# lmdu/pyfastx

Hardware: NVIDIA H100
Metric: index_build_GBps (higher is better)
Workload: dtype u8

## Files before the change

include/fxg.h:

```cpp
#ifndef FXG_H
#define FXG_H
#include <stdint.h>
#ifdef __cplusplus
extern "C" {
#endif

#define FXG_ABI_VERSION 2

enum {
    FXG_OK       = 0,
    FXG_ENODEV   = -1,
    FXG_ECUDA    = -2,
    FXG_EINVAL   = -3,
    FXG_ENOMEM   = -4,
    FXG_ECAP     = -5,
    FXG_EIO      = -6,
    FXG_EFORMAT  = -7
};


typedef struct fxg_fasta_row {
    int64_t boff;
    int64_t blen;
    int64_t slen;
    int64_t llen;
    int32_t dlen;
    int32_t nlen;
    uint8_t elen;
    uint8_t norm;
    uint8_t pad[6];
} fxg_fasta_row;

typedef struct fxg_fastq_row {
    int64_t soff;
    int64_t qoff;
    int64_t rlen;
    int32_t dlen;
    int32_t nlen;
} fxg_fastq_row;

typedef struct fxg_scan_stats {
    int64_t n_rows;
    int64_t n_lines;
    int64_t total_len;
    int64_t end_position;
    int64_t lead_lines;
    int64_t lead_bytes;
    int64_t lead_llen;
    int64_t reserved;
} fxg_scan_stats;

typedef struct fxg_shard_info {
    int64_t n_rows;
    int64_t n_lines;
    int64_t bytes;
    int64_t base_offset;
    int64_t end_position;
    int64_t edge_n;
    int64_t edge_off[3];
    int64_t edge_len[3];
    int64_t reserved[4];
} fxg_shard_info;

enum {
    FXG_SCAN_FULL_NAME = 1
};

enum {
    FXG_X_UPPER      = 1,
    FXG_X_REVERSE    = 2,
    FXG_X_COMPLEMENT = 4,
    FXG_X_RAW        = 8,
    FXG_X_WHOLE      = 16
};

typedef struct fxg_ctx  fxg_ctx;
typedef struct fxg_file fxg_file;
typedef struct fxg_comm fxg_comm;

int         fxg_abi_version(void);
const char *fxg_last_error(void);
int         fxg_device_count(void);
int         fxg_ctx_create(int device, fxg_ctx **out);
void        fxg_ctx_destroy(fxg_ctx *ctx);
int         fxg_ctx_set_stream(fxg_ctx *ctx, void *cuda_stream);
int         fxg_ctx_sync(fxg_ctx *ctx);
int         fxg_ctx_sm_count(fxg_ctx *ctx);

enum { FXG_PROF_SCAN = 0, FXG_PROF_FINALIZE = 1, FXG_PROF_GATHER = 2, FXG_PROF_PLAN = 3, FXG_PROF_PREFIX = 4,
       FXG_PROF_LINES = 5, FXG_PROF_SLOTS = 6 };
int         fxg_profile_enable(fxg_ctx *ctx, int on);
int         fxg_profile_last_ms(fxg_ctx *ctx, int slot, float *ms);
int64_t     fxg_ctx_launch_count(fxg_ctx *ctx);

int         fxg_host_alloc(int64_t nbytes, void **out);
void        fxg_host_free(void *p);

int      fxg_file_alloc(fxg_ctx *ctx, int64_t nbytes, fxg_file **out);
int      fxg_file_upload(fxg_ctx *ctx, fxg_file *f, int64_t dst_off, const void *host, int64_t nbytes);
int      fxg_file_from_host(fxg_ctx *ctx, const void *host, int64_t nbytes, fxg_file **out);
int      fxg_file_from_path(fxg_ctx *ctx, const char *path, fxg_file **out);
int      fxg_file_wrap(fxg_ctx *ctx, void *dev_ptr, int64_t nbytes, int64_t capacity, fxg_file **out);
int      fxg_file_download(fxg_ctx *ctx, const fxg_file *f, int64_t src_off, void *host, int64_t nbytes);
void    *fxg_file_devptr(const fxg_file *f);
int64_t  fxg_file_size(const fxg_file *f);
void     fxg_file_free(fxg_file *f);
void     fxg_pool_trim(void);

int fxg_fasta_scan(fxg_ctx *ctx, const fxg_file *f, int64_t base_offset, int flags,
                   fxg_fasta_row **d_rows_out, fxg_scan_stats *stats);

int fxg_fastq_scan(fxg_ctx *ctx, const fxg_file *f, int64_t base_offset,
                   fxg_fastq_row **d_rows_out, fxg_scan_stats *stats);

int fxg_scan_begin(fxg_ctx *ctx, const fxg_file *f, int mode, int64_t base_offset, int flags,
                   fxg_shard_info *d_info_out );
int fxg_shard_exchange(fxg_ctx *ctx, fxg_comm *comm, const void *d_send, void *d_recv, int64_t bytes_per_rank);
int fxg_scan_finish(fxg_ctx *ctx, const fxg_shard_info *d_all , int nranks, int rank,
                    void **d_rows_out, fxg_scan_stats *stats, fxg_shard_info *all_host);
int fxg_scan_sharded(fxg_ctx *ctx, fxg_comm *comm, const fxg_file *f, int mode, int64_t base_offset, int flags,
                     void **d_rows_out, fxg_scan_stats *stats, fxg_shard_info *all_host);

#define FXG_COMM_ID_BYTES 128
int  fxg_comm_unique_id(void *id_out);
int  fxg_comm_create(fxg_ctx *ctx, const void *id, int nranks, int rank, fxg_comm **out);
int  fxg_comm_nranks(const fxg_comm *comm);
int  fxg_comm_rank(const fxg_comm *comm);
int  fxg_comm_uses_p2p(const fxg_comm *comm);
int  fxg_comm_check(fxg_comm *comm);
void fxg_comm_destroy(fxg_comm *comm);

int fxg_split_point_dev(fxg_ctx *ctx, const fxg_file *f, int64_t from, int want_header, int64_t *pos);
int fxg_split_point_path(const char *path, int64_t from, int want_header, int64_t *pos, int64_t *file_size);
int fxg_file_from_path_range(fxg_ctx *ctx, const char *path, int64_t begin, int64_t end, fxg_file **out);
int fxg_file_slice(fxg_ctx *ctx, const fxg_file *src, int64_t begin, int64_t end, fxg_file **out);

int fxg_rows_download(fxg_ctx *ctx, const void *d_rows, int64_t n_rows, int row_bytes, void *host_rows);
int fxg_rows_upload(fxg_ctx *ctx, const void *host_rows, int64_t n_rows, int row_bytes, void **d_rows_out);
void fxg_dev_free(void *d_ptr);

int fxg_fasta_build_index_host(fxg_ctx *ctx, const void *host_buf, int64_t nbytes, int flags,
                               fxg_fasta_row *rows, int64_t rows_cap, fxg_scan_stats *stats);
int fxg_fastq_build_index_host(fxg_ctx *ctx, const void *host_buf, int64_t nbytes,
                               fxg_fastq_row *rows, int64_t rows_cap, fxg_scan_stats *stats);

int fxg_extract_plan_dev(fxg_ctx *ctx, const int64_t *d_s, const int64_t *d_e, int64_t nq,
                         int64_t *d_out_off, int64_t *total_bytes );
int fxg_extract_dev(fxg_ctx *ctx, const fxg_file *f, const fxg_fasta_row *d_rows, int64_t n_rows,
                    const int64_t *d_row_id, const int64_t *d_s, const int64_t *d_e,
                    const int32_t *d_flags, int64_t nq,
                    const int64_t *d_out_off, uint8_t *d_out, int64_t *d_acgt );
int fxg_extract_host(fxg_ctx *ctx, const fxg_file *f, const fxg_fasta_row *d_rows, int64_t n_rows,
                     const int64_t *row_id, const int64_t *s, const int64_t *e, const int32_t *flags,
                     int64_t nq, int64_t *out_off_host, uint8_t *out_host, int64_t out_cap,
                     int64_t *acgt_host );

int fxg_extract_one_host(fxg_ctx *ctx, const fxg_file *f, const fxg_fasta_row *d_rows, int64_t n_rows,
                         int64_t row_id, int64_t s, int64_t e, int32_t flags, uint8_t *out_host, int64_t out_cap);

int fxg_composition_host(fxg_ctx *ctx, const fxg_file *f, const fxg_fasta_row *d_rows, int64_t n_rows,
                         const int64_t *row_id, const int64_t *s, const int64_t *e, const int32_t *flags,
                         int64_t nq, int64_t *hist_host);

int fxg_reads_dev(fxg_ctx *ctx, const fxg_file *f, const fxg_fastq_row *d_rows, int64_t n_rows,
                  const int64_t *d_ids, int64_t nq, int32_t flags,
                  int64_t *d_out_off, uint8_t *d_seq_out, uint8_t *d_qual_out, int64_t out_cap,
                  int64_t *total_bytes);
int fxg_reads_host(fxg_ctx *ctx, const fxg_file *f, const fxg_fastq_row *d_rows, int64_t n_rows,
                   const int64_t *ids, int64_t nq, int32_t flags,
                   int64_t *out_off_host, uint8_t *seq_host, uint8_t *qual_host, int64_t out_cap);

int fxg_read_one_host(fxg_ctx *ctx, const fxg_file *f, const fxg_fastq_row *d_rows, int64_t n_rows, int64_t read_id,
                      int which, int32_t flags, int64_t rlen, uint8_t *out_host, int64_t out_cap);

int fxg_bgzf_members_host(const void *host_buf, int64_t nbytes, int64_t *cmp_off, int64_t *ucmp_off,
                          int64_t cap, int64_t *n_members, int64_t *total_uncompressed);
int fxg_inflate_members_dev(fxg_ctx *ctx, const fxg_file *compressed, const int64_t *d_cmp_off,
                            const int64_t *d_ucmp_off, int64_t n_members, uint8_t *d_out, int64_t out_cap,
                            int32_t *d_status);
int fxg_file_from_bgzf_host(fxg_ctx *ctx, const void *host_buf, int64_t nbytes, fxg_file **out,
                            int64_t *n_members_out);

typedef struct fxg_gzindex {
    int64_t  compressed_size, uncompressed_size;
    uint32_t spacing, window_size;
    int64_t  npoints;
    const int64_t *cmp_offset;
    const int64_t *uncmp_offset;
    const uint8_t *bits;
    const uint8_t *has_data;
    const uint8_t *windows;
} fxg_gzindex;
typedef struct fxg_comp_row { int64_t seqid, abc, num; } fxg_comp_row;
typedef struct fxg_fastq_meta { int64_t a, c, g, t, n, maxlen, minlen, minqs, maxqs, phred; } fxg_fastq_meta;
int fxg_fxi_write_fasta(const char *path, const fxg_fasta_row *rows, int64_t n_rows, const uint8_t *names,
                        const int64_t *name_off, int64_t total_slen, const fxg_gzindex *gz,
                        const fxg_comp_row *comp, int64_t n_comp);
int fxg_fxi_write_fastq(const char *path, const fxg_fastq_row *rows, int64_t n_rows, const uint8_t *names,
                        const int64_t *name_off, int64_t n_lines, int64_t total_size, const fxg_gzindex *gz,
                        const fxg_fastq_meta *meta);

typedef struct fxg_gzip_result fxg_gzip_result;
int            fxg_gzip_inflate_host(const void *comp, int64_t nbytes, uint32_t spacing , fxg_gzip_result **out);
const uint8_t *fxg_gzip_data(const fxg_gzip_result *r, int64_t *size);
int            fxg_gzip_index(const fxg_gzip_result *r, fxg_gzindex *gz);
void           fxg_gzip_free(fxg_gzip_result *r);
int            fxg_file_from_gzip_points_host(fxg_ctx *ctx, const void *host_buf, int64_t nbytes, const fxg_gzindex *gz,
                                              fxg_file **out);

int  fxg_fasta_composition(fxg_ctx *ctx, const fxg_file *f, const fxg_fasta_row *d_rows, int64_t n_rows,
                           int64_t base_offset, fxg_comp_row **out, int64_t *n_out, int64_t *total );
int  fxg_fastq_stats(fxg_ctx *ctx, const fxg_file *f, const fxg_fastq_row *d_rows, int64_t n_rows,
                     int64_t base_offset, int trailing_seq, fxg_fastq_meta *out);
void fxg_free_host(void *p);

typedef struct fxg_nametab fxg_nametab;
int     fxg_nametab_build(const uint8_t *names, const int64_t *name_off, int64_t n, fxg_nametab **out);
int64_t fxg_nametab_find(const fxg_nametab *t, const uint8_t *name, int64_t len);
int     fxg_nametab_lookup(const fxg_nametab *t, const uint8_t *q, const int64_t *q_off, int64_t nq, int64_t *ids_out);
void    fxg_nametab_free(fxg_nametab *t);

int fxg_bgzf_compress_host(const void *data, int64_t nbytes, int level, uint8_t **out, int64_t *out_len);

int fxg_synth_fasta_dev(fxg_ctx *ctx, uint64_t seed, const int64_t *d_lengths, const int64_t *d_rec_off,
                        int64_t n_records, int64_t first_record, int width, uint8_t *d_out);
int fxg_synth_fastq_dev(fxg_ctx *ctx, uint64_t seed, int64_t n_reads, int64_t first_read, int read_len,
                        const int64_t *d_rec_off, uint8_t *d_out);

#ifdef __cplusplus
}
#endif
#endif
```

pyfastx_b200/_cabi.py:

```python
import ctypes as C
import os
import re

import numpy as np

_HERE = os.path.dirname(os.path.abspath(__file__))
LIB_PATH = os.environ.get("FXG_LIB_PATH") or os.path.join(_HERE, "libfxg.so")
HEADER_PATH = os.path.join(os.path.dirname(_HERE), "include", "fxg.h")

FASTA_ROW = np.dtype([("boff", "<i8"), ("blen", "<i8"), ("slen", "<i8"), ("llen", "<i8"),
                      ("dlen", "<i4"), ("nlen", "<i4"), ("elen", "u1"), ("norm", "u1"),
                      ("pad", "u1", (6,))])
FASTQ_ROW = np.dtype([("soff", "<i8"), ("qoff", "<i8"), ("rlen", "<i8"),
                      ("dlen", "<i4"), ("nlen", "<i4")])

FXG_OK, FXG_ENODEV, FXG_ECUDA, FXG_EINVAL, FXG_ENOMEM, FXG_ECAP, FXG_EIO, FXG_EFORMAT = 0, -1, -2, -3, -4, -5, -6, -7
SCAN_FULL_NAME = 1
X_UPPER, X_REVERSE, X_COMPLEMENT, X_RAW, X_WHOLE = 1, 2, 4, 8, 16


class ScanStats(C.Structure):
    _fields_ = [("n_rows", C.c_int64), ("n_lines", C.c_int64), ("total_len", C.c_int64),
                ("end_position", C.c_int64), ("lead_lines", C.c_int64), ("lead_bytes", C.c_int64),
                ("lead_llen", C.c_int64), ("reserved", C.c_int64)]


class ShardInfo(C.Structure):
    _fields_ = [("n_rows", C.c_int64), ("n_lines", C.c_int64), ("bytes", C.c_int64), ("base_offset", C.c_int64),
                ("end_position", C.c_int64), ("edge_n", C.c_int64), ("edge_off", C.c_int64 * 3),
                ("edge_len", C.c_int64 * 3), ("reserved", C.c_int64 * 4)]


SHARD_INFO = np.dtype([("n_rows", "<i8"), ("n_lines", "<i8"), ("bytes", "<i8"), ("base_offset", "<i8"),
                       ("end_position", "<i8"), ("edge_n", "<i8"), ("edge_off", "<i8", (3,)), ("edge_len", "<i8", (3,)),
                       ("reserved", "<i8", (4,))])
COMM_ID_BYTES = 128


class GzIndex(C.Structure):
    _fields_ = [("compressed_size", C.c_int64), ("uncompressed_size", C.c_int64), ("spacing", C.c_uint32),
                ("window_size", C.c_uint32), ("npoints", C.c_int64), ("cmp_offset", C.c_void_p),
                ("uncmp_offset", C.c_void_p), ("bits", C.c_void_p), ("has_data", C.c_void_p), ("windows", C.c_void_p)]


class FastqMeta(C.Structure):
    _fields_ = [(k, C.c_int64) for k in ("a", "c", "g", "t", "n", "maxlen", "minlen", "minqs", "maxqs", "phred")]


COMP_ROW = np.dtype([("seqid", "<i8"), ("abc", "<i8"), ("num", "<i8")])


class FxgError(RuntimeError):
    def __init__(self, code, msg):
        super().__init__("libfxg error %d: %s" % (code, msg))
        self.code = code


class NoDeviceError(FxgError):
    pass


vp, i64, i32, u64 = C.c_void_p, C.c_int64, C.c_int, C.c_uint64
P = C.POINTER

SIGNATURES = {
    "fxg_abi_version": (i32, []),
    "fxg_last_error": (C.c_char_p, []),
    "fxg_device_count": (i32, []),
    "fxg_ctx_create": (i32, [i32, P(vp)]),
    "fxg_ctx_destroy": (None, [vp]),
    "fxg_ctx_set_stream": (i32, [vp, vp]),
    "fxg_ctx_sync": (i32, [vp]),
    "fxg_ctx_sm_count": (i32, [vp]),
    "fxg_profile_enable": (i32, [vp, i32]),
    "fxg_profile_last_ms": (i32, [vp, i32, P(C.c_float)]),
    "fxg_ctx_launch_count": (i64, [vp]),
    "fxg_host_alloc": (i32, [i64, P(vp)]),
    "fxg_host_free": (None, [vp]),
    "fxg_file_alloc": (i32, [vp, i64, P(vp)]),
    "fxg_file_upload": (i32, [vp, vp, i64, vp, i64]),
    "fxg_file_from_host": (i32, [vp, vp, i64, P(vp)]),
    "fxg_file_from_path": (i32, [vp, C.c_char_p, P(vp)]),
    "fxg_file_wrap": (i32, [vp, vp, i64, i64, P(vp)]),
    "fxg_file_download": (i32, [vp, vp, i64, vp, i64]),
    "fxg_file_devptr": (vp, [vp]),
    "fxg_file_size": (i64, [vp]),
    "fxg_file_free": (None, [vp]),
    "fxg_pool_trim": (None, []),
    "fxg_fasta_scan": (i32, [vp, vp, i64, i32, P(vp), P(ScanStats)]),
    "fxg_fastq_scan": (i32, [vp, vp, i64, P(vp), P(ScanStats)]),
    "fxg_scan_begin": (i32, [vp, vp, i32, i64, i32, vp]),
    "fxg_shard_exchange": (i32, [vp, vp, vp, vp, i64]),
    "fxg_scan_finish": (i32, [vp, vp, i32, i32, P(vp), P(ScanStats), vp]),
    "fxg_scan_sharded": (i32, [vp, vp, vp, i32, i64, i32, P(vp), P(ScanStats), vp]),
    "fxg_comm_unique_id": (i32, [vp]),
    "fxg_comm_create": (i32, [vp, vp, i32, i32, P(vp)]),
    "fxg_comm_nranks": (i32, [vp]),
    "fxg_comm_rank": (i32, [vp]),
    "fxg_comm_uses_p2p": (i32, [vp]),
    "fxg_comm_check": (i32, [vp]),
    "fxg_comm_destroy": (None, [vp]),
    "fxg_split_point_dev": (i32, [vp, vp, i64, i32, P(i64)]),
    "fxg_split_point_path": (i32, [C.c_char_p, i64, i32, P(i64), P(i64)]),
    "fxg_file_from_path_range": (i32, [vp, C.c_char_p, i64, i64, P(vp)]),
    "fxg_file_slice": (i32, [vp, vp, i64, i64, P(vp)]),
    "fxg_rows_download": (i32, [vp, vp, i64, i32, vp]),
    "fxg_rows_upload": (i32, [vp, vp, i64, i32, P(vp)]),
    "fxg_dev_free": (None, [vp]),
    "fxg_fasta_build_index_host": (i32, [vp, vp, i64, i32, vp, i64, P(ScanStats)]),
    "fxg_fastq_build_index_host": (i32, [vp, vp, i64, vp, i64, P(ScanStats)]),
    "fxg_extract_plan_dev": (i32, [vp, vp, vp, i64, vp, P(i64)]),
    "fxg_extract_dev": (i32, [vp, vp, vp, i64, vp, vp, vp, vp, i64, vp, vp, vp]),
    "fxg_extract_host": (i32, [vp, vp, vp, i64, vp, vp, vp, vp, i64, vp, vp, i64, vp]),
    "fxg_extract_one_host": (i32, [vp, vp, vp, i64, i64, i64, i64, i32, vp, i64]),
    "fxg_composition_host": (i32, [vp, vp, vp, i64, vp, vp, vp, vp, i64, vp]),
    "fxg_reads_dev": (i32, [vp, vp, vp, i64, vp, i64, i32, vp, vp, vp, i64, P(i64)]),
    "fxg_reads_host": (i32, [vp, vp, vp, i64, vp, i64, i32, vp, vp, vp, i64]),
    "fxg_read_one_host": (i32, [vp, vp, vp, i64, i64, i32, i32, i64, vp, i64]),
    "fxg_bgzf_members_host": (i32, [vp, i64, vp, vp, i64, P(i64), P(i64)]),
    "fxg_inflate_members_dev": (i32, [vp, vp, vp, vp, i64, vp, i64, vp]),
    "fxg_file_from_bgzf_host": (i32, [vp, vp, i64, P(vp), P(i64)]),
    "fxg_fxi_write_fasta": (i32, [C.c_char_p, vp, i64, vp, vp, i64, vp, vp, i64]),
    "fxg_fxi_write_fastq": (i32, [C.c_char_p, vp, i64, vp, vp, i64, i64, vp, vp]),
    "fxg_gzip_inflate_host": (i32, [vp, i64, C.c_uint32, P(vp)]),
    "fxg_gzip_data": (vp, [vp, P(i64)]),
    "fxg_gzip_index": (i32, [vp, P(GzIndex)]),
    "fxg_gzip_free": (None, [vp]),
    "fxg_file_from_gzip_points_host": (i32, [vp, vp, i64, P(GzIndex), P(vp)]),
    "fxg_fasta_composition": (i32, [vp, vp, vp, i64, i64, P(vp), P(i64), vp]),
    "fxg_fastq_stats": (i32, [vp, vp, vp, i64, i64, i32, P(FastqMeta)]),
    "fxg_free_host": (None, [vp]),
    "fxg_nametab_build": (i32, [vp, vp, i64, P(vp)]),
    "fxg_nametab_find": (i64, [vp, C.c_char_p, i64]),
    "fxg_nametab_lookup": (i32, [vp, vp, vp, i64, vp]),
    "fxg_nametab_free": (None, [vp]),
    "fxg_bgzf_compress_host": (i32, [vp, i64, i32, P(vp), P(i64)]),
    "fxg_synth_fasta_dev": (i32, [vp, u64, vp, vp, i64, i64, i32, vp]),
    "fxg_synth_fastq_dev": (i32, [vp, u64, i64, i64, i32, vp, vp]),
}

_lib = None


def declared_symbols():
    with open(HEADER_PATH) as f:
        text = re.sub(r"/\*.*?\*/", "", f.read(), flags=re.S)
    return sorted(set(re.findall(r"\b(fxg_[a-z0-9_]+)\s*\(", text)))


def lib():
    global _lib
    if _lib is None:
        if not os.path.exists(LIB_PATH):
            raise FxgError(FXG_ENODEV, "libfxg.so not built (run pyfastx_b200/csrc/build.sh or "
                                       "__graft_entry__.build()); there is no CPU fallback")
        L = C.CDLL(LIB_PATH)
        for name, (res, args) in SIGNATURES.items():
            fn = getattr(L, name)
            fn.restype = res
            fn.argtypes = args
        _lib = L
    return _lib


def check(rc):
    if rc != FXG_OK:
        msg = lib().fxg_last_error().decode("utf-8", "replace")
        raise (NoDeviceError if rc == FXG_ENODEV else FxgError)(rc, msg)
    return rc


def ptr(a):
    if a is None:
        return None
    if isinstance(a, int):
        return a
    if isinstance(a, np.ndarray):
        return a.ctypes.data
    if hasattr(a, "data_ptr"):
        return a.data_ptr()
    raise TypeError("cannot take a pointer of %r" % type(a))
```

pyfastx_b200/csrc/fxg_scan.cu:

```cuda
#include "fxg_common.cuh"
#include <stdlib.h>
#include <string.h>
#include <limits.h>

namespace fxg {

#ifndef FXG_MARK_MINB
#define FXG_MARK_MINB 6
#endif
constexpr int REGION   = 2048;
constexpr int SEGCAP   = 128;
constexpr int MARK_WARPS = 8;
constexpr int PS_THREADS = 256, PS_PER_THREAD = 16, PS_BLOCK = PS_THREADS * PS_PER_THREAD;
constexpr int64_t NOPOS = INT64_MIN / 4;
constexpr uint32_t E_POS = 0x07ffu, E_CR = 1u << 14, E_HDR = 1u << 15;

struct __align__(16) FastaTmp {
    int64_t  boff;
    int64_t  lineidx;
    int64_t  llen;
    uint64_t S;
    uint64_t evmax;
    uint64_t evminc;
    uint32_t D;
    int32_t  dlen;
    int32_t  nlen;
    uint32_t elen;
};
static_assert(sizeof(FastaTmp) == 64, "FastaTmp layout");

struct ScanTotals {
    uint64_t nl;
    uint64_t hdr;
    int64_t  n_eff;
    uint64_t sum_len;
    int64_t  lead_lines, lead_bytes, lead_llen;
    int64_t  first_line;
    int64_t  nrows;
    int64_t  row0;
    int64_t  n_owned;
    int64_t  total_lines;
    int64_t  pad[4];
};
static_assert(sizeof(ScanTotals) == 128, "ScanTotals layout");
static_assert(sizeof(fxg_shard_info) == 128, "fxg_shard_info layout");

struct ScanParams;
struct ScanParams {
    const uint8_t *file;
    int64_t   n;
    int64_t   capacity;
    int64_t   nreg;
    int64_t   base_offset;
    int64_t   first_line;
    int       flags;
    uint2    *rc;
    uint4    *rec2;
    uint16_t *seg;
    uint8_t  *cut;
    ulonglong2 *ex;
    ulonglong2 *bs;
    ScanTotals *totals;
    FastaTmp *tmp;
    int64_t   tmp_cap;
    fxg_fastq_row *qrows;
    int64_t   qrows_cap;
    const ScanParams *self;
};

__device__ __forceinline__ uint4 ld_stream16(const uint8_t *p) {
    uint4 v;
    asm volatile("ld.global.nc.L1::no_allocate.v4.u32 {%0, %1, %2, %3}, [%4];"
                 : "=r"(v.x), "=r"(v.y), "=r"(v.z), "=r"(v.w) : "l"(p));
    return v;
}

#ifndef FXG_MARK_CUT
#define FXG_MARK_CUT 0
#endif
#ifndef FXG_CUT_WORDS
#define FXG_CUT_WORDS 6
#endif
__device__ __forceinline__ uint32_t swz_unit(uint32_t u);
template <int V> __device__ __forceinline__ uint32_t region_byte(const uint8_t *sb, uint32_t p);
template <int V>
__device__ __forceinline__ uint32_t name_cut_smem(const uint8_t *sb, uint32_t a) {
    uint32_t M = 0;
#pragma unroll
    for (int k = 0; k < FXG_CUT_WORDS; ++k) {
        const uint32_t wq = min((a >> 2) + (uint32_t)k, (uint32_t)(REGION / 4 - 1));
        const uint32_t w = reinterpret_cast<const uint32_t *>(sb)[V == 2 ? ((swz_unit(wq >> 2) << 2) | (wq & 3u)) : wq];
        const uint32_t lt = ~((((w & 0x7f7f7f7fu) + 0x5f5f5f5fu) | w)) & 0x80808080u;
        M |= ((lt * 0x00204081u) >> 28) << (4 * k);
    }
    M &= 0xffffffffu << (a & 3u);
    if (!M) return 255u;
    const uint32_t p = (a & ~3u) + (uint32_t)(__ffs(M) - 1);
    if (p >= (uint32_t)REGION) return 255u;
    if (p >= ((a >> 2) + (uint32_t)FXG_CUT_WORDS) * 4u) return 255u;
    const uint32_t b = region_byte<V>(sb, p);
    if (b == ' ') return p - a;
    if (b == '\n' || b == 0u) return 254u;
    if (b == '\r' && p + 1u < (uint32_t)REGION && region_byte<V>(sb, p + 1u) == '\n') return 254u;
    return 255u;
}

#ifndef FXG_MARK_V_FASTA
#define FXG_MARK_V_FASTA 1
#endif
#ifndef FXG_MARK_V_FASTQ
#define FXG_MARK_V_FASTQ 2
#endif
#ifndef FXG_MARK_RPW
#define FXG_MARK_RPW 1
#endif
__device__ __forceinline__ uint32_t swz_unit(uint32_t u) { return u ^ ((u >> 3) & 7u); }
template <int V>
__device__ __forceinline__ uint32_t region_byte(const uint8_t *sb, uint32_t p) {
    return V == 2 ? sb[(swz_unit(p >> 4) << 4) | (p & 15u)] : sb[p];
}

template <int MODE, int V>
__global__ void __launch_bounds__(MARK_WARPS * 32, FXG_MARK_MINB) mark_kernel(const ScanParams P) {
    __shared__ uint4    s_data[MARK_WARPS * (REGION / 16) + (FXG_MARK_CUT ? 2 : 0)];
    __shared__ uint16_t s_ent[MARK_WARPS][SEGCAP];
    const int lane = threadIdx.x & 31, warp = threadIdx.x >> 5;
    const int64_t r0 = ((int64_t)blockIdx.x * MARK_WARPS + warp) * FXG_MARK_RPW;
    if (r0 >= P.nreg) return;
    const uint32_t lt_mask = (1u << lane) - 1u;
    const int64_t n = P.n;
    const uint8_t *file = P.file;
    const uint32_t k0a = reg_const(0x0a0a0a0au), k7f = reg_const(0x7f7f7f7fu), k80 = reg_const(0x80808080u);

    auto load_region = [&](int64_t rr, uint4 (&vv)[4]) {
        const int64_t base = rr * REGION;
        if (base + REGION <= n) {
            const uint8_t *src = file + base + lane * 16;
#pragma unroll
            for (int j = 0; j < 4; ++j) vv[j] = ld_stream16(src + j * 512);
        } else {
#pragma unroll
            for (int j = 0; j < 4; ++j) {
                const int64_t o = base + j * 512 + lane * 16;
                if (o + 16 <= n) { vv[j] = ld_stream16(file + o); continue; }
                const bool virt = n > 0 && file[n - 1] != '\n';
                uint32_t w[4] = {0, 0, 0, 0};
                for (int i = 0; i < 16; ++i) {
                    const int64_t x = o + i;
                    const uint32_t b = x < n ? file[x] : ((virt && x == n) ? 0x0au : 0u);
                    w[i >> 2] |= b << ((i & 3) * 8);
                }
                vv[j] = make_uint4(w[0], w[1], w[2], w[3]);
            }
        }
    };
    uint4 vn[4];
    load_region(r0, vn);
#pragma unroll 1
    for (int it = 0; it < FXG_MARK_RPW; ++it) {
    const int64_t r = r0 + it;
    if (r >= P.nreg) break;
    const int64_t base = r * REGION;
    uint4 v[4] = {vn[0], vn[1], vn[2], vn[3]};
    if (it + 1 < FXG_MARK_RPW && r + 1 < P.nreg) load_region(r + 1, vn);
    uint32_t nlc = 0;
    uint16_t *ent = s_ent[warp];

    if constexpr (V == 2) {
    uint4 *sd = s_data + warp * (REGION / 16);
#pragma unroll
    for (int j = 0; j < 4; ++j) sd[swz_unit((uint32_t)(j * 32 + lane))] = v[j];
    __syncwarp();
    uint32_t lo = 0, hi = 0;
#pragma unroll
    for (int i = 0; i < 4; ++i) {
        const uint4 x = sd[swz_unit((uint32_t)(4 * lane + i))];
        const uint32_t w4[4] = {x.x, x.y, x.z, x.w};
#pragma unroll
        for (int c = 0; c < 4; ++c) {
            const uint32_t f = byte_eq_mask_r(w4[c], k0a, k7f, k80);
            const uint32_t nib = (f * 0x00204081u) >> 28;
            const int k = 4 * i + c;
            if (k < 8) lo = nib * (1u << (4 * k)) + lo;
            else hi = nib * (1u << (4 * (k - 8))) + hi;
        }
    }
    {
        const uint32_t c = (uint32_t)(__popc(lo) + __popc(hi));
        const uint32_t b1 = __ballot_sync(0xffffffffu, c >= 1u), b2 = __ballot_sync(0xffffffffu, c >= 2u);
        const uint32_t b3 = __ballot_sync(0xffffffffu, c >= 3u);
        const uint32_t pbase = (uint32_t)lane * 64u;
        if (!b3) {
            const uint32_t idx = (uint32_t)(__popc(b1 & lt_mask) + __popc(b2 & lt_mask));
            nlc = (uint32_t)(__popc(b1) + __popc(b2));
            if (c) {
                const uint32_t p1 = lo ? (uint32_t)(__ffs(lo) - 1) : 32u + (uint32_t)(__ffs(hi) - 1);
                if (idx < (uint32_t)SEGCAP) ent[idx] = (uint16_t)(pbase + p1);
                if (c >= 2u) {
                    if (lo) lo &= lo - 1u; else hi &= hi - 1u;
                    const uint32_t p2 = lo ? (uint32_t)(__ffs(lo) - 1) : 32u + (uint32_t)(__ffs(hi) - 1);
                    if (idx + 1u < (uint32_t)SEGCAP) ent[idx + 1u] = (uint16_t)(pbase + p2);
                }
            }
        } else {
            uint32_t incl = c;
#pragma unroll
            for (int d = 1; d < 32; d <<= 1) {
                const uint32_t o2 = __shfl_up_sync(0xffffffffu, incl, d);
                if (lane >= d) incl += o2;
            }
            nlc = __shfl_sync(0xffffffffu, incl, 31);
            uint32_t idx = incl - c;
            while (lo) { if (idx < (uint32_t)SEGCAP) ent[idx] = (uint16_t)(pbase + (uint32_t)(__ffs(lo) - 1)); lo &= lo - 1u; ++idx; }
            while (hi) { if (idx < (uint32_t)SEGCAP) ent[idx] = (uint16_t)(pbase + 32u + (uint32_t)(__ffs(hi) - 1)); hi &= hi - 1u; ++idx; }
        }
    }
    __syncwarp();
    } else {
    uint32_t m[4];
    int cmax = 0;
#pragma unroll
    for (int j = 0; j < 4; ++j) {
        s_data[warp * (REGION / 16) + j * 32 + lane] = v[j];
        m[j] = chunk_eq_mask_r(v[j], k0a, k7f, k80);
        cmax = max(cmax, __popc(m[j]));
    }
    const bool any2 = __any_sync(0xffffffffu, cmax >= 2);
    const bool multi = any2 && __any_sync(0xffffffffu, cmax >= 3);
    if (!any2) {
#pragma unroll
        for (int j = 0; j < 4; ++j) {
            const uint32_t bn = __ballot_sync(0xffffffffu, m[j] != 0);
            if (m[j]) {
                const uint32_t idx = nlc + __popc(bn & lt_mask);
                if (idx < (uint32_t)SEGCAP) ent[idx] = (uint16_t)(j * 512 + lane * 16 + chunk_bit_to_off(__ffs(m[j]) - 1));
            }
            nlc += __popc(bn);
        }
    } else if (!multi) {
#pragma unroll
        for (int j = 0; j < 4; ++j) {
            const int c = __popc(m[j]);
            const uint32_t bn1 = __ballot_sync(0xffffffffu, c >= 1);
            const uint32_t bn2 = __ballot_sync(0xffffffffu, c >= 2);
            if (c) {
                const uint32_t idx = nlc + __popc(bn1 & lt_mask) + __popc(bn2 & lt_mask);
                const int xo = j * 512 + lane * 16;
                int oa = chunk_bit_to_off(__ffs(m[j]) - 1);
                if (c == 2) {
                    const uint32_t m2 = m[j] & (m[j] - 1);
                    const int ob = chunk_bit_to_off(__ffs(m2) - 1);
                    const int hi = max(oa, ob);
                    oa = min(oa, ob);
                    if (idx + 1 < (uint32_t)SEGCAP) ent[idx + 1] = (uint16_t)(xo + hi);
                }
                if (idx < (uint32_t)SEGCAP) ent[idx] = (uint16_t)(xo + oa);
            }
            nlc += __popc(bn1) + __popc(bn2);
        }
    }
    if (multi) {
        nlc = 0;
#pragma unroll 1
        for (int j = 0; j < 4; ++j) {
            uint32_t mj = 0;
#pragma unroll
            for (int jj = 0; jj < 4; ++jj) if (jj == j) mj = m[jj];
            const uint32_t c = (uint32_t)__popc(mj);
            uint32_t incl = c;
#pragma unroll
            for (int d = 1; d < 32; d <<= 1) {
                const uint32_t o2 = __shfl_up_sync(0xffffffffu, incl, d);
                if (lane >= d) incl += o2;
            }
            uint32_t idx = nlc + incl - c;
#pragma unroll 1
            for (int w = 0; w < 4; ++w) {
                uint32_t mw = mj & (0x80808080u >> w);
                while (mw) {
                    if (idx < (uint32_t)SEGCAP) ent[idx] = (uint16_t)(j * 512 + lane * 16 + chunk_bit_to_off(__ffs(mw) - 1));
                    mw &= mw - 1;
                    ++idx;
                }
            }
            nlc += __shfl_sync(0xffffffffu, incl, 31);
        }
    }
    __syncwarp();
    }

    const uint8_t *sb = reinterpret_cast<const uint8_t *>(s_data + warp * (REGION / 16));
    uint32_t hc = 0;
    if (nlc <= (uint32_t)SEGCAP) {
        uint16_t *dst = P.seg + r * SEGCAP;
        const uint32_t nround = (nlc + 15u) & ~15u;
        uint32_t imask = 0, hmask = 0;
        for (uint32_t k0 = 0; k0 < nround; k0 += 32) {
            const uint32_t k = k0 + lane;
            uint32_t e = 0, cutv = 255u;
            if (k < nlc) {
                const uint32_t pos = ent[k];
                e = pos;
                if (FXG_MARK_CUT && MODE == 1 && pos + 2u < (uint32_t)REGION && region_byte<V>(sb, pos + 1u) == '@') cutv = name_cut_smem<V>(sb, pos + 2u);
                if (MODE == 0) {
                    const uint32_t next = pos < (uint32_t)(REGION - 1) ? region_byte<V>(sb, pos + 1u)
                                                                      : (base + REGION < n ? (uint32_t)file[base + REGION] : 0u);
                    if (next == '>') e |= E_HDR;
                } else {
                    const uint32_t prev = pos > 0 ? region_byte<V>(sb, pos - 1u) : (base > 0 ? (uint32_t)file[base - 1] : 0u);
                    if (prev == '\r') e |= E_CR;
                }
            }
            if (MODE == 0) {
                const uint32_t hb = __ballot_sync(0xffffffffu, (e & E_HDR) != 0);
                hc += __popc(hb);
                if (k0 == 0) {
                    const uint32_t e1 = __shfl_up_sync(0xffffffffu, e, 1), e2 = __shfl_up_sync(0xffffffffu, e, 2);
                    const bool it = lane >= 2 && k < nlc &&
                                    (((e1 | e2) & E_HDR) != 0 || (e & E_POS) - (e1 & E_POS) != (e1 & E_POS) - (e2 & E_POS));
                    imask = __ballot_sync(0xffffffffu, it);
                    hmask = hb;
                }
            }
            if (k < nround) dst[k] = (uint16_t)e;
            if (FXG_MARK_CUT && MODE == 1) P.cut[r * SEGCAP + k] = (uint8_t)cutv;
            if (k < nlc) ent[k] = (uint16_t)e;
        }
        __syncwarp();
        if (lane == 0) {
            const uint32_t last = nlc >= 1 ? ent[nlc - 1] : 0u, prev = nlc >= 2 ? ent[nlc - 2] : 0u;
            P.rc[r] = make_uint2(nlc | (hc << 16), last | (prev << 16));
            if (MODE == 0) {
                const uint32_t f0 = nlc >= 1 ? ent[0] : 0u, f1 = nlc >= 2 ? ent[1] : 0u;
                P.rec2[r] = make_uint4(f0 | (f1 << 16), nlc > 32u ? 0xffffffffu : imask, hmask, 0u);
            }
        }
    } else {
        if (MODE == 0) {
            uint32_t myh = 0;
            for (int x = lane; x < REGION; x += 32)
                if (region_byte<V>(sb, (uint32_t)x) == '\n') {
                    const uint32_t next = x < REGION - 1 ? region_byte<V>(sb, (uint32_t)x + 1u) : (base + REGION < n ? (uint32_t)file[base + REGION] : 0u);
                    myh += next == '>';
                }
            hc = __reduce_add_sync(0xffffffffu, myh);
        }
        if (lane == 0) {
            P.rc[r] = make_uint2(nlc | (hc << 16), 0u);
            if (MODE == 0) P.rec2[r] = make_uint4(0u, 0xffffffffu, 0u, 0u);
        }
    }
    __syncwarp();
    }
}

__global__ void __launch_bounds__(PS_THREADS) prefix_reduce_kernel(const uint2 *rc, ulonglong2 *bs) {
    __shared__ uint32_t sm[16];
    const uint4 *p = reinterpret_cast<const uint4 *>(rc + (size_t)blockIdx.x * PS_BLOCK + (size_t)threadIdx.x * PS_PER_THREAD);
    uint32_t a = 0, b = 0;
#pragma unroll
    for (int i = 0; i < PS_PER_THREAD / 2; ++i) {
        const uint4 q = p[i];
        a += (q.x & 0xffffu) + (q.z & 0xffffu);
        b += (q.x >> 16) + (q.z >> 16);
    }
    a = __reduce_add_sync(0xffffffffu, a);
    b = __reduce_add_sync(0xffffffffu, b);
    const int lane = threadIdx.x & 31, warp = threadIdx.x >> 5;
    if (lane == 0) { sm[warp] = a; sm[8 + warp] = b; }
    __syncthreads();
    if (threadIdx.x == 0) {
        uint64_t ta = 0, tb = 0;
        for (int w = 0; w < PS_THREADS / 32; ++w) { ta += sm[w]; tb += sm[8 + w]; }
        bs[blockIdx.x] = make_ulonglong2(ta, tb);
    }
}

__global__ void __launch_bounds__(1024) prefix_blocks_kernel(ulonglong2 *bs, int64_t nb, const uint8_t *file, int64_t n,
                                                             int mode, ScanTotals *tot) {
    __shared__ uint64_t s_a[32], s_b[32];
    __shared__ uint64_t s_ca, s_cb;
    const int lane = threadIdx.x & 31, warp = threadIdx.x >> 5;
    if (threadIdx.x == 0) { s_ca = 0; s_cb = (mode == 0 && n > 0 && file[0] == '>') ? 1u : 0u; }
    __syncthreads();
    for (int64_t b0 = 0; b0 < nb; b0 += 1024) {
        const int64_t i = b0 + threadIdx.x;
        const ulonglong2 v = i < nb ? bs[i] : make_ulonglong2(0, 0);
        uint64_t a = v.x, b = v.y;
#pragma unroll
        for (int d = 1; d < 32; d <<= 1) {
            const uint64_t oa = (uint64_t)shfl_up_i64((int64_t)a, d), ob = (uint64_t)shfl_up_i64((int64_t)b, d);
            if (lane >= d) { a += oa; b += ob; }
        }
        if (lane == 31) { s_a[warp] = a; s_b[warp] = b; }
        __syncthreads();
        uint64_t wa = 0, wb = 0;
        for (int w = 0; w < warp; ++w) { wa += s_a[w]; wb += s_b[w]; }
        const uint64_t ca = s_ca, cb = s_cb;
        if (i < nb) bs[i] = make_ulonglong2(ca + wa + a - v.x, cb + wb + b - v.y);
        __syncthreads();
        if (threadIdx.x == 1023) { s_ca = ca + wa + a; s_cb = cb + wb + b; }
        __syncthreads();
    }
    if (threadIdx.x == 0) {
        const bool virt = n > 0 && file[n - 1] != '\n';
        tot->nl = s_ca; tot->hdr = s_cb; tot->n_eff = n + (virt ? 1 : 0);
    }
}

__global__ void __launch_bounds__(PS_THREADS) prefix_expand_kernel(const uint2 *rc, const ulonglong2 *bs, ulonglong2 *ex,
                                                                 int64_t nreg) {
    __shared__ uint32_t s_a[PS_THREADS / 32], s_b[PS_THREADS / 32];
    const int lane = threadIdx.x & 31, warp = threadIdx.x >> 5;
    const size_t r0 = (size_t)blockIdx.x * PS_BLOCK + (size_t)threadIdx.x * PS_PER_THREAD;
    const uint4 *p = reinterpret_cast<const uint4 *>(rc + r0);
    uint32_t c[PS_PER_THREAD];
    uint32_t a = 0, b = 0;
#pragma unroll
    for (int i = 0; i < PS_PER_THREAD / 2; ++i) {
        const uint4 q = p[i];
        c[2 * i] = q.x; c[2 * i + 1] = q.z;
        a += (q.x & 0xffffu) + (q.z & 0xffffu);
        b += (q.x >> 16) + (q.z >> 16);
    }
    uint32_t ia = a, ib = b;
#pragma unroll
    for (int d = 1; d < 32; d <<= 1) {
        const uint32_t oa = __shfl_up_sync(0xffffffffu, ia, d), ob = __shfl_up_sync(0xffffffffu, ib, d);
        if (lane >= d) { ia += oa; ib += ob; }
    }
    if (lane == 31) { s_a[warp] = ia; s_b[warp] = ib; }
    __syncthreads();
    uint32_t wa = 0, wb = 0;
    for (int w = 0; w < warp; ++w) { wa += s_a[w]; wb += s_b[w]; }
    const ulonglong2 bb = bs[blockIdx.x];
    uint64_t ea = bb.x + wa + ia - a, eb = bb.y + wb + ib - b;
#pragma unroll
    for (int i = 0; i < PS_PER_THREAD; ++i) {
        if ((int64_t)(r0 + i) < nreg) ex[r0 + i] = make_ulonglong2(ea, eb);
        ea += c[i] & 0xffffu; eb += c[i] >> 16;
    }
}

__device__ __forceinline__ int64_t find_first_of2(const uint8_t *h, int64_t limit, uint32_t a4, uint32_t b4, int *which) {
    const int mis = (int)((uintptr_t)h & 3);
    const uint32_t *wp = reinterpret_cast<const uint32_t *>(h - mis);
    *which = 0;
    for (int64_t k = -mis; k < limit; k += 16, wp += 4) {
        const uint32_t w0 = wp[0], w1 = wp[1], w2 = wp[2], w3 = wp[3];
        uint32_t ma[4] = {byte_eq_mask(w0, a4), byte_eq_mask(w1, a4), byte_eq_mask(w2, a4), byte_eq_mask(w3, a4)};
        uint32_t mb[4] = {byte_eq_mask(w0, b4), byte_eq_mask(w1, b4), byte_eq_mask(w2, b4), byte_eq_mask(w3, b4)};
#pragma unroll
        for (int i = 0; i < 4; ++i) {
            uint32_t m = ma[i] | mb[i];
            const int64_t kk = k + 4 * i;
            if (kk < 0) m &= 0xffffffffu << (8 * (int)(-kk));
            if (m) {
                const int byte = (__ffs(m) - 1) >> 3;
                const int64_t pos = kk + byte;
                if (pos >= limit) return limit;
                *which = ((mb[i] >> (8 * byte)) & 0x80u) ? 2 : 1;
                return pos;
            }
        }
    }
    return limit;
}

struct Prev2 {
    int64_t  pos1, pos0;
    uint32_t h1, h0;
};

template <int MODE>
__device__ __forceinline__ uint32_t is_hdr_at(const ScanParams &P, int64_t x) {
    return (MODE == 0 && x < P.n && P.file[x] == '>') ? 1u : 0u;
}
__device__ __forceinline__ bool nl_at(const ScanParams &P, int64_t x) {
    return x < P.n ? P.file[x] == '\n' : (x == P.n && P.n > 0 && P.file[P.n - 1] != '\n');
}

template <int MODE>
__device__ __forceinline__ void do_line(const ScanParams &P, int64_t first_line, int64_t p, int64_t pm1, int64_t pm2, bool h1, bool h2,
                                        int64_t hcount, int64_t lineidx, bool cr, unsigned long long &my_size) {
    const uint8_t *file = P.file;
    const int64_t s = pm1 + 1;
    const int64_t L = p - pm1;
    if (MODE == 0) {
        const int64_t slot = hcount;
        if (h1) {
            const int elen = (p >= 1 && (p - 1 < P.n ? file[p - 1] : 0) == '\r') ? 2 : 1;
            const int64_t dlen = L - 1 - elen;
            int64_t nlen = dlen;
            if (!(P.flags & FXG_SCAN_FULL_NAME)) {
                nlen = 0;
                if (s + 1 + dlen + 20 <= P.capacity) {
                    int which;
                    nlen = find_first_of2(file + s + 1, dlen, 0x20202020u, 0x09090909u, &which);
                } else {
                    while (nlen < dlen) {
                        const uint8_t ch = file[s + 1 + nlen];
                        if (ch == ' ' || ch == '\t') break;
                        ++nlen;
                    }
                }
            }
            if (slot < P.tmp_cap) {
                FastaTmp *t = &P.tmp[slot];
                t->boff = P.base_offset + p + 1;
                t->lineidx = lineidx;
                t->dlen = (int32_t)dlen;
                t->nlen = (int32_t)nlen;
                t->elen = (uint32_t)elen;
            }
        } else if (slot < P.tmp_cap) {
            const bool prev_exists = pm1 >= 0;
            if (!prev_exists || h2) {
                P.tmp[slot].llen = L;
            } else {
                const int64_t prevL = pm1 - pm2;
                if (L != prevL) {
                    FastaTmp *t = &P.tmp[slot];
                    atomicAdd(&t->D, 1u);
                    atomicMax((unsigned long long *)&t->evmax, (unsigned long long)lineidx);
                    atomicMax((unsigned long long *)&t->evminc, ~(unsigned long long)lineidx);
                    atomicAdd((unsigned long long *)&t->S, (unsigned long long)(L - prevL));
                }
            }
        }
    } else {
        const int64_t gline = first_line + lineidx;
        const int ph = (int)(gline & 3);
        const int64_t row = (gline >> 2) - (first_line >> 2);
        const int64_t len = L - 1;
        if (ph == 1) {
            const int64_t rlen = (len > 0 && cr) ? len - 1 : len;
            my_size += (unsigned long long)rlen;
            if (row < P.qrows_cap) { P.qrows[row].soff = P.base_offset + s; P.qrows[row].rlen = rlen; }
        } else if (row < P.qrows_cap) {
            if (ph == 0) {
                int64_t l = len - 1;
                if (l > 0 && cr) --l;
                if (l < 0) l = 0;
                int64_t k = 0;
                if (s + 1 + l + 20 <= P.capacity) {
                    int which;
                    k = find_first_of2(file + s + 1, l, 0x20202020u, 0x00000000u, &which);
                    if (which == 2) k = l;
                } else {
                    for (; k < l; ++k) {
                        const uint8_t ch = file[s + 1 + k];
                        if (ch == 0) { k = l; break; }
                        if (ch == ' ') break;
                    }
                }
                *reinterpret_cast<int2 *>(&P.qrows[row].dlen) = make_int2((int)len, (int)k);
            } else if (ph == 3) {
                P.qrows[row].qoff = P.base_offset + s;
            }
        }
    }
}

template <int MODE>
__device__ __noinline__ Prev2 carry_walk(const ScanParams *Pg, int64_t r) {
    const ScanParams &P = *Pg;
    Prev2 cy;
    const int lane = threadIdx.x & 31;
    cy.pos1 = cy.pos0 = NOPOS; cy.h1 = cy.h0 = 0;
    int need = 2;
    auto push = [&](int64_t pos, uint32_t h) {
        if (need == 2) { cy.pos1 = pos; cy.h1 = h; } else { cy.pos0 = pos; cy.h0 = h; }
        --need;
    };
    int64_t q = r - 1;
    while (need > 0 && q >= 0) {
        const int64_t qq = q - lane;
        const uint32_t c = qq >= 0 ? (P.rc[qq].x & 0xffffu) : 0u;
        const uint32_t nz = __ballot_sync(0xffffffffu, c != 0);
        if (!nz) { q -= 32; continue; }
        const int f = __ffs(nz) - 1;
        q -= f;
        const int cq = (int)__shfl_sync(0xffffffffu, c, f);
        if (cq <= SEGCAP) {
            const uint16_t *sg = P.seg + q * SEGCAP;
            for (int i = cq - 1; i >= 0 && need > 0; --i) {
                const uint32_t e = sg[i];
                push(q * REGION + (int64_t)(e & E_POS), MODE == 0 ? (e >> 15) : 0u);
            }
        } else {
            for (int64_t x = q * REGION + REGION - 1; x >= q * REGION && need > 0; --x)
                if (nl_at(P, x)) push(x, is_hdr_at<MODE>(P, x + 1));
        }
        q -= 1;
    }
    if (need > 0) push(-1, is_hdr_at<MODE>(P, 0));
    return cy;
}

template <int MODE>
__device__ __noinline__ unsigned long long dense_region(const ScanParams *Pg, int64_t first_line, int64_t r, Prev2 cy,
                                                        ulonglong2 exv) {
    const ScanParams &P = *Pg;
    unsigned long long my_size = 0;
    const int lane = threadIdx.x & 31;
    const uint8_t *file = P.file;
    const int64_t b0 = r * REGION + lane * 64;
    uint32_t c = 0, h = 0;
    Prev2 inc; inc.pos1 = inc.pos0 = NOPOS; inc.h1 = inc.h0 = 0;
    for (int i = 0; i < 64; ++i) {
        const int64_t x = b0 + i;
        if (nl_at(P, x)) {
            const uint32_t hh = is_hdr_at<MODE>(P, x + 1);
            ++c; h += hh;
            inc.pos0 = inc.pos1; inc.h0 = inc.h1; inc.pos1 = x; inc.h1 = hh;
        }
    }
    uint32_t ic = c, ih = h;
    uint32_t icnt = c > 2 ? 2 : c;
#pragma unroll
    for (int d = 1; d < 32; d <<= 1) {
        const uint32_t oc = __shfl_up_sync(0xffffffffu, ic, d), oh = __shfl_up_sync(0xffffffffu, ih, d);
        const int64_t op1 = shfl_up_i64(inc.pos1, d), op0 = shfl_up_i64(inc.pos0, d);
        const uint32_t oh1 = __shfl_up_sync(0xffffffffu, inc.h1, d), oh0 = __shfl_up_sync(0xffffffffu, inc.h0, d);
        const uint32_t ocnt = __shfl_up_sync(0xffffffffu, icnt, d);
        if (lane >= d) {
            ic += oc; ih += oh;
            if (icnt == 0) { inc.pos1 = op1; inc.h1 = oh1; inc.pos0 = op0; inc.h0 = oh0; icnt = ocnt; }
            else if (icnt == 1 && ocnt >= 1) { inc.pos0 = op1; inc.h0 = oh1; icnt = 2; }
        }
    }
    Prev2 pv;
    pv.pos1 = shfl_up_i64(inc.pos1, 1); pv.pos0 = shfl_up_i64(inc.pos0, 1);
    pv.h1 = __shfl_up_sync(0xffffffffu, inc.h1, 1); pv.h0 = __shfl_up_sync(0xffffffffu, inc.h0, 1);
    uint32_t pcnt = __shfl_up_sync(0xffffffffu, icnt, 1);
    if (lane == 0) pcnt = 0;
    if (pcnt == 0) pv = cy;
    else if (pcnt == 1) { pv.pos0 = cy.pos1; pv.h0 = cy.h1; }
    int64_t idx = (int64_t)exv.x + (ic - c);
    int64_t hcount = (int64_t)exv.y + (ih - h);
    for (int i = 0; i < 64 && c; ++i) {
        const int64_t x = b0 + i;
        if (!nl_at(P, x)) continue;
        const bool cr = x > 0 && file[x - 1] == '\r';
        do_line<MODE>(P, first_line, x, pv.pos1, pv.pos0, pv.h1 != 0, pv.h0 != 0, hcount, idx, cr, my_size);
        const uint32_t hh = is_hdr_at<MODE>(P, x + 1);
        hcount += hh; ++idx;
        pv.pos0 = pv.pos1; pv.h0 = pv.h1; pv.pos1 = x; pv.h1 = hh;
    }
    return my_size;
}

template <int MODE>
__device__ __forceinline__ void region_batches(const ScanParams &P, int64_t first_line, int64_t r, int nl, Prev2 cy, ulonglong2 X,
                                               uint32_t E0, uint32_t E1, unsigned long long &my_size) {
    const int lane = threadIdx.x & 31;
    const uint32_t lt_mask = (1u << lane) - 1u;
    const int64_t base = r * REGION;
    const uint16_t *sg = P.seg + r * SEGCAP;
    int64_t hrun = (int64_t)X.y;
    for (int k0 = 0; k0 < nl; k0 += 32) {
        const int k = k0 + lane;
        const bool valid = k < nl;
        uint32_t e = k0 == 0 ? E0 : (k0 == 32 ? E1 : (valid ? (uint32_t)sg[k] : 0u));
        if (!valid) e = 0;
        const uint32_t hb = __ballot_sync(0xffffffffu, (e & E_HDR) != 0);
        const uint32_t e1 = __shfl_up_sync(0xffffffffu, e, 1), e2 = __shfl_up_sync(0xffffffffu, e, 2);
        if (valid) {
            int64_t pm1, pm2;
            bool h1, h2;
            if (lane >= 1) { pm1 = base + (e1 & E_POS); h1 = (e1 & E_HDR) != 0; } else { pm1 = cy.pos1; h1 = cy.h1 != 0; }
            if (lane >= 2) { pm2 = base + (e2 & E_POS); h2 = (e2 & E_HDR) != 0; }
            else if (lane == 1) { pm2 = cy.pos1; h2 = cy.h1 != 0; }
            else { pm2 = cy.pos0; h2 = cy.h0 != 0; }
            do_line<MODE>(P, first_line, base + (e & E_POS), pm1, pm2, h1, h2, hrun + __popc(hb & lt_mask), (int64_t)X.x + k,
                          (e & E_CR) != 0, my_size);
        }
        const uint32_t l31 = __shfl_sync(0xffffffffu, e, 31), l30 = __shfl_sync(0xffffffffu, e, 30);
        cy.pos1 = base + (l31 & E_POS); cy.h1 = (l31 >> 15) & 1u;
        cy.pos0 = base + (l30 & E_POS); cy.h0 = (l30 >> 15) & 1u;
        hrun += __popc(hb);
    }
}

template <int MODE>
__device__ __noinline__ unsigned long long full_region(const ScanParams *Pg, int64_t first_line, int64_t r) {
    const ScanParams &P = *Pg;
    unsigned long long my_size = 0;
    const int lane = threadIdx.x & 31;
    const int nl = (int)(P.rc[r].x & 0xffffu);
    if (nl == 0) return 0;
    const ulonglong2 X = P.ex[r];
    Prev2 cy = carry_walk<MODE>(Pg, r);
    if (MODE != 0) cy.h1 = cy.h0 = 0;
    if (nl <= SEGCAP) region_batches<MODE>(P, first_line, r, nl, cy, X, P.seg[r * SEGCAP + lane], P.seg[r * SEGCAP + 32 + lane], my_size);
    else my_size += dense_region<MODE>(Pg, first_line, r, cy, X);
    return my_size;
}

constexpr int LG = 4;

template <int MODE>
__global__ void __launch_bounds__(MARK_WARPS * 32) lines_kernel(const ScanParams P) {
    const int64_t first_line = MODE == 1 ? P.totals->first_line : 0;
    const int lane = threadIdx.x & 31;
    const int64_t r0 = ((int64_t)blockIdx.x * MARK_WARPS + (threadIdx.x >> 5)) * LG;
    if (r0 >= P.nreg) return;
    unsigned long long my_size = 0;

    const int64_t rq = r0 + (LG - 1) - lane;
    const uint2 A = rq >= 0 ? P.rc[rq] : make_uint2(0u, 0u);
    ulonglong2 X[LG];
    uint32_t E[LG][2];
#pragma unroll
    for (int i = 0; i < LG; ++i) {
        const int64_t r = r0 + i;
        X[i] = make_ulonglong2(0, 0); E[i][0] = E[i][1] = 0;
        if (r < P.nreg) {
            X[i] = P.ex[r];
            E[i][0] = P.seg[r * SEGCAP + lane];
            E[i][1] = P.seg[r * SEGCAP + 32 + lane];
        }
    }
    const uint32_t cntl = A.x & 0xffffu;
    const uint32_t nzall = __ballot_sync(0xffffffffu, cntl != 0);
    const bool window_hits_start = r0 + (LG - 1) - 31 <= 0;

#pragma unroll
    for (int i = 0; i < LG; ++i) {
        const int64_t r = r0 + i;
        const int me = LG - 1 - i;
        const int nl = (int)__shfl_sync(0xffffffffu, cntl, me);
        if (nl == 0) continue;

        Prev2 cy;
        cy.pos1 = cy.pos0 = NOPOS; cy.h1 = cy.h0 = 0;
        {
            bool slow = false;
            const uint32_t nz = nzall & ~((2u << me) - 1u);
            if (nz) {
                const int f1 = __ffs(nz) - 1;
                const uint32_t n1 = __shfl_sync(0xffffffffu, cntl, f1), y1 = __shfl_sync(0xffffffffu, A.y, f1);
                const int64_t b1 = (r0 + (LG - 1) - f1) * REGION;
                if (n1 > (uint32_t)SEGCAP) slow = true;
                else {
                    cy.pos1 = b1 + (y1 & E_POS); cy.h1 = (y1 >> 15) & 1u;
                    if (n1 >= 2) { cy.pos0 = b1 + ((y1 >> 16) & E_POS); cy.h0 = y1 >> 31; }
                    else {
                        const uint32_t nz2 = nz & ~(1u << f1);
                        if (nz2) {
                            const int f2 = __ffs(nz2) - 1;
                            const uint32_t n2 = __shfl_sync(0xffffffffu, cntl, f2), y2 = __shfl_sync(0xffffffffu, A.y, f2);
                            if (n2 > (uint32_t)SEGCAP) slow = true;
                            else { cy.pos0 = (r0 + (LG - 1) - f2) * REGION + (y2 & E_POS); cy.h0 = (y2 >> 15) & 1u; }
                        } else if (window_hits_start) { cy.pos0 = -1; cy.h0 = is_hdr_at<MODE>(P, 0); }
                        else slow = true;
                    }
                }
            } else if (window_hits_start) { cy.pos1 = -1; cy.h1 = is_hdr_at<MODE>(P, 0); }
            else slow = true;
            if (slow) cy = carry_walk<MODE>(P.self, r);
            if (MODE != 0) cy.h1 = cy.h0 = 0;
        }
        if (nl <= SEGCAP) region_batches<MODE>(P, first_line, r, nl, cy, X[i], E[i][0], E[i][1], my_size);
        else my_size += dense_region<MODE>(P.self, first_line, r, cy, X[i]);
    }

    if (MODE == 1) {
#pragma unroll
        for (int d = 16; d > 0; d >>= 1) my_size += (unsigned long long)shfl_down_i64((int64_t)my_size, d);
        if (lane == 0 && my_size) atomicAdd((unsigned long long *)&P.totals->sum_len, my_size);
    }
}

#ifndef FXG_FQ_PRELOAD
#define FXG_FQ_PRELOAD 0
#endif
#ifndef FXG_FQ_PAIRSTORE
#define FXG_FQ_PAIRSTORE 1
#endif
constexpr int RG = 8;
constexpr int RWIN = RG + 2;
static_assert(RWIN * REGION <= 32768, "window positions must fit 15 bits");

__global__ void __launch_bounds__(MARK_WARPS * 32) fastq_records_kernel(const ScanParams Pin) {
    __shared__ uint16_t s_flat[MARK_WARPS][RWIN * SEGCAP];
    __shared__ uint8_t  s_cut[MARK_WARPS][FXG_MARK_CUT ? RWIN * SEGCAP : 1];
    const ScanParams &P = Pin;
    const int64_t first_line = Pin.totals->first_line;
    const int lane = threadIdx.x & 31, warp = threadIdx.x >> 5;
    const int64_t r0 = ((int64_t)blockIdx.x * MARK_WARPS + warp) * RG;
    if (r0 >= P.nreg) return;
    unsigned long long my_size = 0;
    const uint8_t *file = P.file;

    const int64_t rl = r0 - 1 + lane;
    uint2 rec = make_uint2(0u, 0u);
    uint64_t exl = 0;
    if (lane <= RWIN && rl >= 0 && rl < P.nreg) { rec = P.rc[rl]; exl = P.ex[rl].x; }
    const uint32_t nll = rec.x & 0xffffu;
    const uint32_t densem = __ballot_sync(0xffffffffu, nll > (uint32_t)SEGCAP);
    if (densem & (((1u << RG) - 1u) << 1)) {
        for (int i = 0; i < RG; ++i)
            if (r0 + i < P.nreg) my_size += full_region<1>(P.self, first_line, r0 + i);
    } else {
        const uint64_t ex0 = (uint64_t)shfl_i64((int64_t)exl, 1);
        uint16_t *flat = s_flat[warp];
        uint8_t *cutf = s_cut[warp];
        uint32_t E2[RWIN];
#pragma unroll
        for (int i = 0; i < RWIN; ++i) {
            E2[i] = 0u;
            if (FXG_FQ_PRELOAD && r0 + i < P.nreg) E2[i] = reinterpret_cast<const uint32_t *>(P.seg + (r0 + i) * SEGCAP)[lane];
        }
        int W = 0, Ls = 0;
        bool closed = false;
#pragma unroll
        for (int i = 0; i < RWIN; ++i) {
            const int nl = (int)__shfl_sync(0xffffffffu, nll, i + 1);
            if (nl > SEGCAP) closed = true;
            if (!closed) {
                const int k = 2 * lane;
                if (!FXG_FQ_PRELOAD && k < nl) E2[i] = reinterpret_cast<const uint32_t *>(P.seg + (r0 + i) * SEGCAP)[lane];
                const uint32_t e0 = E2[i] & 0xffffu, e1 = E2[i] >> 16;
                if (k < nl) flat[W + k] = (uint16_t)((i * REGION + (int)(e0 & E_POS)) | ((e0 & E_CR) ? 0x8000u : 0u));
                if (k + 1 < nl) flat[W + k + 1] = (uint16_t)((i * REGION + (int)(e1 & E_POS)) | ((e1 & E_CR) ? 0x8000u : 0u));
                if (nl > 64) {
                    const uint16_t *sg = P.seg + (r0 + i) * SEGCAP;
                    for (int kk = 64 + lane; kk < nl; kk += 32) {
                        const uint32_t e = sg[kk];
                        flat[W + kk] = (uint16_t)((i * REGION + (int)(e & E_POS)) | ((e & E_CR) ? 0x8000u : 0u));
                    }
                }
                if (FXG_MARK_CUT) {
                    const uint8_t *cg = P.cut + (r0 + i) * SEGCAP;
                    for (int kk = lane; kk < nl; kk += 32) cutf[W + kk] = cg[kk];
                }
                W += nl;
            }
            if (i == RG - 1) Ls = W;
        }
        __syncwarp();
        int64_t carry;
        uint32_t carry_cut = 255u;
        {
            const uint32_t pn = __shfl_sync(0xffffffffu, nll, 0), py = __shfl_sync(0xffffffffu, rec.y, 0);
            if (r0 == 0) carry = -1;
            else if (pn >= 1 && pn <= (uint32_t)SEGCAP) {
                carry = (r0 - 1) * REGION + (int64_t)(py & E_POS);
                if (FXG_MARK_CUT) carry_cut = P.cut[(r0 - 1) * SEGCAP + (pn - 1)];
            } else carry = carry_walk<1>(P.self, r0).pos1;
        }
        const int64_t span_base = r0 * REGION;
        auto POS = [&](int f) -> int64_t { return f < 0 ? carry : span_base + (int64_t)(flat[f] & 0x7fffu); };
        auto CR = [&](int f) -> bool { return (flat[f] & 0x8000u) != 0; };
        const int64_t g0 = first_line + (int64_t)ex0;
        const int64_t row0 = first_line >> 2;
        int lead = (int)((4 - (g0 & 3)) & 3);
        if (lead > Ls) lead = Ls;
        if (lane < lead) {
            const int f = lane;
            const int64_t g = g0 + f;
            const int ph = (int)(g & 3);
            const int64_t row = (g >> 2) - row0;
            const int64_t pm1 = POS(f - 1), p = POS(f);
            if (ph == 1) {
                const int64_t len = p - pm1 - 1;
                const int64_t rlen = (len > 0 && CR(f)) ? len - 1 : len;
                my_size += (unsigned long long)rlen;
                if (row < P.qrows_cap) { P.qrows[row].soff = P.base_offset + pm1 + 1; P.qrows[row].rlen = rlen; }
            } else if (ph == 3) {
                if (row < P.qrows_cap) P.qrows[row].qoff = P.base_offset + pm1 + 1;
            }
        }
        for (int fb = lead; fb < Ls; fb += 128) {
            const int f = fb + 4 * lane;
            int64_t row = 0, soff = 0, rlen = 0, qoff = 0, len = 0, k = 0;
            bool have1 = false, have3 = false;
            const bool mine = f < Ls;
            if (mine) {
                row = ((g0 + f) >> 2) - row0;
                have1 = f + 1 < W; have3 = f + 3 < W;
                const int64_t pm1 = POS(f - 1), p0 = POS(f);
                len = p0 - pm1 - 1;
                int64_t l = len - 1;
                if (l > 0 && CR(f)) --l;
                if (l < 0) l = 0;
                const int64_t s = pm1 + 1;
                const uint32_t cv = !FXG_MARK_CUT ? 255u : (f >= 1 ? (uint32_t)cutf[f - 1] : carry_cut);
                if (cv < 254u) k = (int64_t)cv < l ? (int64_t)cv : l;
                else if (cv == 254u) k = l;
                else if (s + 1 + l + 20 <= P.capacity) {
                    int which;
                    k = find_first_of2(file + s + 1, l, 0x20202020u, 0x00000000u, &which);
                    if (which == 2) k = l;
                } else {
                    for (; k < l; ++k) {
                        const uint8_t ch = file[s + 1 + k];
                        if (ch == 0) { k = l; break; }
                        if (ch == ' ') break;
                    }
                }
                if (have1) {
                    const int64_t p1 = POS(f + 1);
                    const int64_t len1 = p1 - p0 - 1;
                    soff = P.base_offset + p0 + 1;
                    rlen = (len1 > 0 && CR(f + 1)) ? len1 - 1 : len1;
                    if (f + 1 < Ls) my_size += (unsigned long long)rlen;
                }
                if (have3) qoff = P.base_offset + POS(f + 2) + 1;
            }
            const bool full = mine && have3 && row < P.qrows_cap;
            const int other_full = __shfl_xor_sync(0xffffffffu, full ? 1 : 0, 1);
            const bool pair_full = FXG_FQ_PAIRSTORE && full && other_full != 0;
            longlong2 a, b;
            a.x = soff; a.y = qoff;
            b.x = rlen; b.y = (long long)(((unsigned long long)(uint32_t)(int)k << 32) | (uint32_t)(int)len);
            const bool odd = (lane & 1) != 0;
            const longlong2 send = odd ? a : b;
            longlong2 recv;
            recv.x = shfl_i64(send.x, lane ^ 1);
            recv.y = shfl_i64(send.y, lane ^ 1);
            if (pair_full) {
                fxg_fastq_row *q0 = &P.qrows[odd ? row - 1 : row];
                reinterpret_cast<longlong2 *>(q0)[odd ? 1 : 0] = odd ? recv : a;
                reinterpret_cast<longlong2 *>(q0 + 1)[odd ? 1 : 0] = odd ? b : recv;
            } else if (mine && row < P.qrows_cap) {
                fxg_fastq_row *q = &P.qrows[row];
                if (have3) {
                    reinterpret_cast<longlong2 *>(q)[0] = a;
                    reinterpret_cast<longlong2 *>(q)[1] = b;
                } else {
                    *reinterpret_cast<int2 *>(&q->dlen) = make_int2((int)len, (int)k);
                    if (have1) { q->soff = soff; q->rlen = rlen; }
                }
            }
        }
    }
#pragma unroll
    for (int d = 16; d > 0; d >>= 1) my_size += (unsigned long long)shfl_down_i64((int64_t)my_size, d);
    if (lane == 0 && my_size) atomicAdd((unsigned long long *)&P.totals->sum_len, my_size);
}

__global__ void __launch_bounds__(MARK_WARPS * 32) fasta_lines_kernel(const ScanParams P) {
    const int lane = threadIdx.x & 31;
    const int64_t R0 = ((int64_t)blockIdx.x * MARK_WARPS + (threadIdx.x >> 5)) * 32;
    if (R0 >= P.nreg) return;
    const int64_t r = R0 + lane;
    const bool inb = r < P.nreg;
    unsigned long long dummy = 0;
    uint2 me = make_uint2(0u, 0u), pv = make_uint2(0u, 0u);
    uint4 q = make_uint4(0u, 0u, 0u, 0u);
    ulonglong2 X = make_ulonglong2(0, 0);
    if (inb) {
        me = P.rc[r];
        if (r >= 1) pv = P.rc[r - 1];
        q = P.rec2[r];
        X = P.ex[r];
    }
    const uint32_t nl = me.x & 0xffffu, pnl = pv.x & 0xffffu;
    const bool full = nl != 0 && (nl > 32u || r == 0 || pnl < 2u || pnl > (uint32_t)SEGCAP || q.y == 0xffffffffu);
    uint32_t mask = 0;
    const uint32_t c1 = pv.y & 0xffffu, c0 = pv.y >> 16, f0 = q.x & 0xffffu, f1 = q.x >> 16;
    if (nl != 0 && !full) {
        const int p_c1 = (int)(c1 & E_POS) - REGION, p_c0 = (int)(c0 & E_POS) - REGION;
        const int p_f0 = (int)(f0 & E_POS), p_f1 = (int)(f1 & E_POS);
        const int L0 = p_f0 - p_c1;
        const bool i0 = ((c1 | c0) & E_HDR) != 0 || L0 != p_c1 - p_c0;
        const bool i1 = nl >= 2u && (((f0 | c1) & E_HDR) != 0 || p_f1 - p_f0 != L0);
        mask = (q.y & ~3u) | (i0 ? 1u : 0u) | (i1 ? 2u : 0u);
        if (nl < 32u) mask &= (1u << nl) - 1u;
    }
    const int64_t base = r * REGION;
    const uint16_t *sg = P.seg + r * SEGCAP;
    while (mask) {
        const int k = __ffs(mask) - 1;
        mask &= mask - 1;
        uint32_t e, m1, m2;
        int64_t b1 = base, b2 = base;
        if (k >= 2) { e = sg[k]; m1 = sg[k - 1]; m2 = sg[k - 2]; }
        else if (k == 1) { e = f1; m1 = f0; m2 = c1; b2 = base - REGION; }
        else { e = f0; m1 = c1; m2 = c0; b1 = b2 = base - REGION; }
        do_line<0>(P, 0, base + (e & E_POS), b1 + (m1 & E_POS), b2 + (m2 & E_POS), (m1 & E_HDR) != 0, (m2 & E_HDR) != 0,
                   (int64_t)X.y + __popc(q.z & ((1u << k) - 1u)), (int64_t)X.x + k, false, dummy);
    }
    uint32_t fm = __ballot_sync(0xffffffffu, full);
    while (fm) {
        const int f = __ffs(fm) - 1;
        fm &= fm - 1;
        full_region<0>(P.self, 0, R0 + f);
    }
}


__global__ void __launch_bounds__(256) fasta_finalize_kernel(const FastaTmp *tmp, int64_t tmp_cap, int64_t rows_cap,
                                                             int64_t base_offset, ScanTotals *tot, fxg_fasta_row *rows) {
    int64_t nrows = (int64_t)tot->hdr;
    if (nrows > rows_cap || nrows + 1 > tmp_cap) nrows = 0;
    unsigned long long slen_acc = 0;
    const int64_t stride = (int64_t)gridDim.x * blockDim.x;
    for (int64_t r = (int64_t)blockIdx.x * blockDim.x + threadIdx.x; r < nrows; r += stride) {
        const FastaTmp t = tmp[r + 1];
        int64_t next_h, next_line;
        if (r + 1 < nrows) {
            const FastaTmp nx = tmp[r + 2];
            next_h = nx.boff - (1 + nx.dlen + (int64_t)nx.elen);
            next_line = nx.lineidx;
        } else {
            next_h = base_offset + tot->n_eff;
            next_line = (int64_t)tot->nl;
        }
        const int64_t blen = next_h - t.boff;
        const int64_t nlines = next_line - t.lineidx - 1;
        const int64_t slen = blen - nlines * (int64_t)t.elen;
        int norm;
        if (t.D == 0) norm = 1;
        else if (t.D == 1) norm = ((int64_t)t.evmax == t.lineidx + nlines) ? 1 : 0;
        else if (t.D == 2) norm = ((t.evmax - (~t.evminc) == 1) && t.S == 0) ? 1 : 0;
        else norm = 0;
        fxg_fasta_row o;
        o.boff = t.boff; o.blen = blen; o.slen = slen; o.llen = t.llen;
        o.dlen = t.dlen; o.nlen = t.nlen; o.elen = (uint8_t)t.elen; o.norm = (uint8_t)norm;
        for (int i = 0; i < 6; ++i) o.pad[i] = 0;
        o.pad[0] = (t.D == 0 || (t.D == 1 && (int64_t)t.evmax == t.lineidx + nlines && (int64_t)t.S < 0)) ? 1 : 0;
        rows[r] = o;
        slen_acc += (unsigned long long)slen;
    }
#pragma unroll
    for (int d = 16; d > 0; d >>= 1) slen_acc += (unsigned long long)shfl_down_i64((int64_t)slen_acc, d);
    if ((threadIdx.x & 31) == 0 && slen_acc) atomicAdd((unsigned long long *)&tot->sum_len, slen_acc);
    if (blockIdx.x == 0 && threadIdx.x == 0) {
        const FastaTmp l = tmp[0];
        tot->lead_llen = l.llen;
        if (nrows > 0) {
            const FastaTmp f = tmp[1];
            tot->lead_lines = f.lineidx;
            tot->lead_bytes = f.boff - base_offset - (1 + f.dlen + (int64_t)f.elen);
        }
    }
}

__global__ void __launch_bounds__(32) edge_kernel(const ScanParams P, int mode, fxg_shard_info *info) {
    const int lane = threadIdx.x;
    int found = 0;
    int64_t pos[3] = {0, 0, 0};
    for (int64_t r0 = 0; r0 < P.nreg && found < 3; r0 += 32) {
        const int64_t r = r0 + lane;
        const uint32_t c = r < P.nreg ? (P.rc[r].x & 0xffffu) : 0u;
        uint32_t nz = __ballot_sync(0xffffffffu, c != 0);
        while (nz && found < 3) {
            const int fl = __ffs(nz) - 1;
            nz &= nz - 1;
            const int64_t q = r0 + fl;
            const int cq = (int)__shfl_sync(0xffffffffu, c, fl);
            if (cq <= SEGCAP) {
                for (int i = 0; i < cq && found < 3; ++i) pos[found++] = q * REGION + (int64_t)(P.seg[q * SEGCAP + i] & E_POS);
            } else {
                for (int64_t x = q * REGION; x < q * REGION + REGION && found < 3; ++x)
                    if (nl_at(P, x)) pos[found++] = x;
            }
        }
    }
    if (lane == 0) {
        const ScanTotals t = *P.totals;
        fxg_shard_info o;
        o.n_rows = mode == 0 ? (int64_t)t.hdr : 0;
        o.n_lines = (int64_t)t.nl;
        o.bytes = P.n;
        o.base_offset = P.base_offset;
        o.end_position = t.n_eff;
        o.edge_n = found;
        int64_t start = 0;
        for (int j = 0; j < 3; ++j) {
            o.edge_off[j] = 0; o.edge_len[j] = 0;
            if (j < found) {
                const int64_t p = pos[j];
                const bool cr = p > start && p - 1 < P.n && P.file[p - 1] == '\r';
                o.edge_off[j] = P.base_offset + start;
                o.edge_len[j] = p - start - (cr ? 1 : 0);
                start = p + 1;
            }
        }
        for (int j = 0; j < 4; ++j) o.reserved[j] = 0;
        *info = o;
    }
}

__global__ void shard_prefix_kernel(const fxg_shard_info *all, int nranks, int rank, int mode, ScanTotals *tot) {
    if (threadIdx.x != 0 || blockIdx.x != 0) return;
    int64_t F = 0, T = 0;
    for (int p = 0; p < nranks; ++p) {
        const int64_t nlp = all[p].n_lines;
        if (p < rank) F += nlp;
        T += nlp;
    }
    if (mode == 0) F = 0;
    tot->first_line = F;
    tot->total_lines = T;
    const int64_t nl = (int64_t)tot->nl;
    tot->nrows = mode == 0 ? (int64_t)tot->hdr : (F + nl + 3) / 4 - F / 4;
    tot->sum_len = 0;
}

__global__ void __launch_bounds__(256) clear_kernel(const ScanParams P, int mode, int64_t tmp_slots) {
    const int64_t nrows = P.totals->nrows;
    const int64_t stride = (int64_t)gridDim.x * blockDim.x;
    const int64_t t0 = (int64_t)blockIdx.x * blockDim.x + threadIdx.x;
    if (mode == 0) {
        int64_t slots = nrows + 2;
        if (slots > tmp_slots) slots = tmp_slots;
        uint4 *p = reinterpret_cast<uint4 *>(P.tmp);
        for (int64_t i = t0; i < slots * 4; i += stride) p[i] = make_uint4(0u, 0u, 0u, 0u);
    } else if (t0 < 4) {
        const int64_t row = t0 < 2 ? 0 : nrows - 1;
        if (row >= 0 && row < P.qrows_cap) reinterpret_cast<uint4 *>(P.qrows + row)[t0 & 1] = make_uint4(0u, 0u, 0u, 0u);
    }
}

__global__ void fastq_stitch_kernel(const ScanParams P, const fxg_shard_info *all, int nranks, int rank) {
    if (threadIdx.x != 0 || blockIdx.x != 0) return;
    ScanTotals *tot = P.totals;
    const int64_t F = tot->first_line, n = (int64_t)tot->nl, T = tot->total_lines;
    const int64_t first_read = (F + 3) / 4;
    int64_t last_read = n > 0 ? (F + n - 1) / 4 : first_read - 1;
    if (last_read > T / 4 - 1) last_read = T / 4 - 1;
    const int64_t owned = last_read >= first_read ? last_read - first_read + 1 : 0;
    tot->row0 = first_read - F / 4;
    tot->n_owned = owned;
    if (owned == 0) return;
    const int64_t row = last_read - F / 4;
    if (row >= P.qrows_cap) return;
    for (int ph = 1; ph <= 3; ph += 2) {
        const int64_t g = 4 * last_read + ph;
        if (g < F + n) continue;
        int64_t Fp = F + n;
        for (int p = rank + 1; p < nranks; ++p) {
            const int64_t np = all[p].n_lines;
            if (g < Fp + np) {
                const int64_t j = g - Fp;
                if (j < all[p].edge_n) {
                    if (ph == 1) { P.qrows[row].soff = all[p].edge_off[j]; P.qrows[row].rlen = all[p].edge_len[j]; }
                    else P.qrows[row].qoff = all[p].edge_off[j];
                }
                break;
            }
            Fp += np;
        }
    }
}

__global__ void __launch_bounds__(256) split_point_kernel(const uint8_t *file, int64_t n, int64_t from, int want_header,
                                                          long long *out) {
    __shared__ long long s_best;
    if (threadIdx.x == 0) s_best = LLONG_MAX;
    __syncthreads();
    if (from <= 0) {
        if (!want_header || (n > 0 && file[0] == '>')) { if (threadIdx.x == 0) *out = 0; return; }
        from = 1;
    }
    for (int64_t c0 = from - 1; c0 < n; c0 += 256 * 16) {
        const int64_t a = c0 + threadIdx.x * 16;
        long long mine = LLONG_MAX;
        for (int i = 0; i < 16; ++i) {
            const int64_t x = a + i;
            if (x < n && file[x] == '\n' && (!want_header || (x + 1 < n && file[x + 1] == '>'))) { mine = x + 1; break; }
        }
        if (mine != LLONG_MAX) atomicMin(&s_best, mine);
        __syncthreads();
        if (s_best != LLONG_MAX) break;
        __syncthreads();
    }
    if (threadIdx.x == 0) *out = s_best == LLONG_MAX ? n : s_best;
}

}

using namespace fxg;

static int64_t guess_rows(int mode, int64_t n) { return (mode == 0 ? n / 1024 : n / 200) + 4096; }

static int scan_params(fxg_ctx *ctx, const fxg_file *f, int mode, int64_t base_offset, int flags, bool reserve,
                       ScanParams *out, int64_t *tmp_slots) {
    const int64_t n = f->size;
    const int64_t nreg = (n + 1 + REGION - 1) / REGION;
    const int64_t nb = (nreg + PS_BLOCK - 1) / PS_BLOCK;
    const int64_t nreg_pad = nb * PS_BLOCK;
    const size_t off_bs = fxg_round_up((int64_t)nreg_pad * 8, 256);
    const size_t off_ex = off_bs + fxg_round_up(nb * (int64_t)sizeof(ulonglong2), 256);
    const size_t off_r2 = off_ex + fxg_round_up(nreg * (int64_t)sizeof(ulonglong2), 256);
    int rc;
    if (reserve) {
        if ((rc = ctx->counters.reserve(1024))) return rc;
        if ((rc = ctx->tile_desc.reserve(off_r2 + (mode == 0 ? (size_t)nreg * sizeof(uint4) : 0)))) return rc;
        if ((rc = ctx->seg.reserve((size_t)nreg * SEGCAP * sizeof(uint16_t)))) return rc;
        if (FXG_MARK_CUT && mode == 1 && (rc = ctx->cut.reserve((size_t)nreg * SEGCAP))) return rc;
        const int64_t want = guess_rows(mode, n);
        if (mode == 0) {
            if (ctx->row_tmp.cap < (size_t)(want + 2) * sizeof(FastaTmp) && (rc = ctx->row_tmp.reserve((size_t)(want + 2) * sizeof(FastaTmp)))) return rc;
            if (ctx->rows.cap < (size_t)(want + 1) * sizeof(fxg_fasta_row) && (rc = ctx->rows.reserve((size_t)(want + 1) * sizeof(fxg_fasta_row)))) return rc;
        } else if (ctx->rows.cap < (size_t)(want + 2) * sizeof(fxg_fastq_row)) {
            if ((rc = ctx->rows.reserve((size_t)(want + 2) * sizeof(fxg_fastq_row)))) return rc;
        }
    }
    ScanParams P;
    memset(&P, 0, sizeof(P));
    P.file = f->d; P.n = n; P.capacity = f->capacity & ~(int64_t)15; P.nreg = nreg;
    P.base_offset = base_offset; P.first_line = 0; P.flags = flags;
    P.rc = (uint2 *)ctx->tile_desc.ptr;
    P.bs = (ulonglong2 *)((uint8_t *)ctx->tile_desc.ptr + off_bs);
    P.ex = (ulonglong2 *)((uint8_t *)ctx->tile_desc.ptr + off_ex);
    P.rec2 = (uint4 *)((uint8_t *)ctx->tile_desc.ptr + off_r2);
    P.seg = (uint16_t *)ctx->seg.ptr;
    P.cut = (uint8_t *)ctx->cut.ptr;
    P.totals = (ScanTotals *)((uint8_t *)ctx->counters.ptr + 64);
    *tmp_slots = 0;
    if (mode == 0) {
        *tmp_slots = (int64_t)(ctx->row_tmp.cap / sizeof(FastaTmp));
        P.tmp = (FastaTmp *)ctx->row_tmp.ptr;
        P.tmp_cap = *tmp_slots - 1;
    } else {
        P.qrows = (fxg_fastq_row *)ctx->rows.ptr;
        P.qrows_cap = (int64_t)(ctx->rows.cap / sizeof(fxg_fastq_row));
    }
    *out = P;
    return FXG_OK;
}

static fxg_shard_info *own_info(fxg_ctx *ctx) { return (fxg_shard_info *)((uint8_t *)ctx->counters.ptr + 256); }

extern "C" int fxg_scan_begin(fxg_ctx *ctx, const fxg_file *f, int mode, int64_t base_offset, int flags,
                              fxg_shard_info *d_info_out) {
    FXG_CHECK_ARG(ctx && f && (mode == 0 || mode == 1), "null ctx/file or bad mode");
    FXG_LOCK(ctx);
    FXG_CUDA(cudaSetDevice(ctx->device));
    ctx->run.active = false;
    ScanParams P;
    int64_t tmp_slots;
    int rc = scan_params(ctx, f, mode, base_offset, flags, true, &P, &tmp_slots);
    if (rc) return rc;
    const int64_t n = f->size, nreg = P.nreg;
    const int64_t nb = (nreg + PS_BLOCK - 1) / PS_BLOCK, nreg_pad = nb * PS_BLOCK;
    FXG_CUDA(cudaMemsetAsync(ctx->counters.ptr, 0, 1024, ctx->stream));
    if (nreg_pad > nreg) FXG_CUDA(cudaMemsetAsync(P.rc + nreg, 0, (size_t)(nreg_pad - nreg) * 8, ctx->stream));
    const unsigned grid = (unsigned)((nreg + (int64_t)MARK_WARPS * FXG_MARK_RPW - 1) / ((int64_t)MARK_WARPS * FXG_MARK_RPW));
    {
        FxgProfScope prof(ctx, FXG_PROF_SCAN);
        if (mode == 0) mark_kernel<0, FXG_MARK_V_FASTA><<<grid, MARK_WARPS * 32, 0, ctx->stream>>>(P);
        else mark_kernel<1, FXG_MARK_V_FASTQ><<<grid, MARK_WARPS * 32, 0, ctx->stream>>>(P);
    }
    FXG_CUDA(cudaGetLastError());
    {
        FxgProfScope prof(ctx, FXG_PROF_PREFIX, 4);
        prefix_reduce_kernel<<<(unsigned)nb, PS_THREADS, 0, ctx->stream>>>(P.rc, P.bs);
        prefix_blocks_kernel<<<1, 1024, 0, ctx->stream>>>(P.bs, nb, P.file, n, mode, P.totals);
        prefix_expand_kernel<<<(unsigned)nb, PS_THREADS, 0, ctx->stream>>>(P.rc, P.bs, P.ex, nreg);
        edge_kernel<<<1, 32, 0, ctx->stream>>>(P, mode, own_info(ctx));
    }
    FXG_CUDA(cudaGetLastError());
    if (d_info_out)
        FXG_CUDA(cudaMemcpyAsync(d_info_out, own_info(ctx), sizeof(fxg_shard_info), cudaMemcpyDeviceToDevice, ctx->stream));
    ctx->run.active = true; ctx->run.mode = mode; ctx->run.flags = flags; ctx->run.file = f; ctx->run.base_offset = base_offset;
    return FXG_OK;
}

static int launch_phase_b(fxg_ctx *ctx, const ScanParams &P0, int mode, int64_t tmp_slots, const fxg_shard_info *d_all,
                          int nranks, int rank) {
    int rc0 = ctx->params.reserve(512);
    if (rc0) return rc0;
    if (!ctx->h_counters) FXG_CUDA(cudaHostAlloc(&ctx->h_counters, 8192, cudaHostAllocDefault));
    ScanParams P = P0;
    P.self = (const ScanParams *)ctx->params.ptr;
    static_assert(sizeof(ScanParams) <= 512, "ScanParams staging");
    memcpy((uint8_t *)ctx->h_counters + 4096, &P, sizeof(P));
    FXG_CUDA(cudaMemcpyAsync(ctx->params.ptr, (uint8_t *)ctx->h_counters + 4096, sizeof(P), cudaMemcpyHostToDevice, ctx->stream));
    const int64_t nreg = P.nreg;
    {
        FxgProfScope prof(ctx, FXG_PROF_LINES, 3);
        shard_prefix_kernel<<<1, 32, 0, ctx->stream>>>(d_all, nranks, rank, mode, P.totals);
        clear_kernel<<<ctx->sm_count * 4, 256, 0, ctx->stream>>>(P, mode, tmp_slots);
        if (mode == 0) {
            const unsigned lgrid = (unsigned)((nreg + MARK_WARPS * 32 - 1) / (MARK_WARPS * 32));
            fasta_lines_kernel<<<lgrid, MARK_WARPS * 32, 0, ctx->stream>>>(P);
        } else if (getenv("FXG_FASTQ_LINES_GENERIC")) {
            const unsigned lgrid = (unsigned)((nreg + MARK_WARPS * LG - 1) / (MARK_WARPS * LG));
            lines_kernel<1><<<lgrid, MARK_WARPS * 32, 0, ctx->stream>>>(P);
        } else {
            const unsigned lgrid = (unsigned)((nreg + MARK_WARPS * RG - 1) / (MARK_WARPS * RG));
            fastq_records_kernel<<<lgrid, MARK_WARPS * 32, 0, ctx->stream>>>(P);
        }
    }
    FXG_CUDA(cudaGetLastError());
    {
        FxgProfScope prof(ctx, FXG_PROF_FINALIZE);
        if (mode == 0)
            fasta_finalize_kernel<<<ctx->sm_count * 4, 256, 0, ctx->stream>>>(
                P.tmp, P.tmp_cap, (int64_t)(ctx->rows.cap / sizeof(fxg_fasta_row)), P.base_offset, P.totals,
                (fxg_fasta_row *)ctx->rows.ptr);
        else
            fastq_stitch_kernel<<<1, 32, 0, ctx->stream>>>(P, d_all, nranks, rank);
    }
    FXG_CUDA(cudaGetLastError());
    return FXG_OK;
}

extern "C" int fxg_scan_finish(fxg_ctx *ctx, const fxg_shard_info *d_all, int nranks, int rank, void **d_rows_out,
                               fxg_scan_stats *stats, fxg_shard_info *all_host) {
    FXG_CHECK_ARG(ctx && stats && nranks >= 1 && rank >= 0 && rank < nranks, "bad arguments");
    FXG_LOCK(ctx);
    FXG_CHECK_ARG(ctx->run.active, "fxg_scan_finish without fxg_scan_begin");
    FXG_CUDA(cudaSetDevice(ctx->device));
    ctx->run.active = false;
    const int mode = ctx->run.mode;
    const fxg_file *f = ctx->run.file;
    if (!d_all) { FXG_CHECK_ARG(nranks == 1, "d_all == NULL with more than one rank"); d_all = own_info(ctx); }
    memset(stats, 0, sizeof(*stats));
    if (d_rows_out) *d_rows_out = nullptr;
    if (!ctx->h_counters) FXG_CUDA(cudaHostAlloc(&ctx->h_counters, 8192, cudaHostAllocDefault));
    FXG_CHECK_ARG((size_t)nranks * sizeof(fxg_shard_info) + 256 <= 4096 || !all_host, "too many ranks for all_host");
    ScanTotals *ht = (ScanTotals *)ctx->h_counters;
    fxg_shard_info *hall = (fxg_shard_info *)((uint8_t *)ctx->h_counters + 256);
    for (int attempt = 0; attempt < 2; ++attempt) {
        ScanParams P;
        int64_t tmp_slots;
        int rc = scan_params(ctx, f, mode, ctx->run.base_offset, ctx->run.flags, false, &P, &tmp_slots);
        if (rc) return rc;
        if ((rc = launch_phase_b(ctx, P, mode, tmp_slots, d_all, nranks, rank))) return rc;
        FXG_CUDA(cudaMemcpyAsync(ht, P.totals, sizeof(ScanTotals), cudaMemcpyDeviceToHost, ctx->stream));
        if (all_host)
            FXG_CUDA(cudaMemcpyAsync(hall, d_all, (size_t)nranks * sizeof(fxg_shard_info), cudaMemcpyDeviceToHost, ctx->stream));
        FXG_CUDA(cudaStreamSynchronize(ctx->stream));
        bool fits;
        if (mode == 0) fits = ht->nrows + 2 <= tmp_slots && (size_t)(ht->nrows + 1) * sizeof(fxg_fasta_row) <= ctx->rows.cap;
        else fits = ht->nrows <= P.qrows_cap;
        if (fits) break;
        if (attempt == 1) { fxg_set_error("row buffers still too small after regrowing"); return FXG_ENOMEM; }
        if (mode == 0) {
            if ((rc = ctx->row_tmp.reserve((size_t)(ht->nrows + 2) * sizeof(FastaTmp)))) return rc;
            if ((rc = ctx->rows.reserve((size_t)(ht->nrows + 1) * sizeof(fxg_fasta_row)))) return rc;
        } else if ((rc = ctx->rows.reserve((size_t)(ht->nrows + 2) * sizeof(fxg_fastq_row)))) return rc;
    }
    stats->n_lines = (int64_t)ht->nl;
    stats->end_position = ht->n_eff;
    stats->total_len = (int64_t)ht->sum_len;
    if (mode == 0) {
        stats->n_rows = ht->nrows;
        stats->lead_llen = ht->lead_llen;
        if (ht->nrows > 0) { stats->lead_lines = ht->lead_lines; stats->lead_bytes = ht->lead_bytes; }
        else { stats->lead_lines = (int64_t)ht->nl; stats->lead_bytes = f->size; }
        if (d_rows_out) *d_rows_out = ctx->rows.ptr;
    } else {
        stats->n_rows = ht->n_owned;
        stats->lead_lines = ht->first_line;
        stats->reserved = ht->total_lines;
        if (d_rows_out) *d_rows_out = (fxg_fastq_row *)ctx->rows.ptr + ht->row0;
    }
    if (all_host) memcpy(all_host, hall, (size_t)nranks * sizeof(fxg_shard_info));
    return FXG_OK;
}

extern "C" int fxg_scan_sharded(fxg_ctx *ctx, fxg_comm *comm, const fxg_file *f, int mode, int64_t base_offset, int flags,
                                void **d_rows_out, fxg_scan_stats *stats, fxg_shard_info *all_host) {
    FXG_CHECK_ARG(ctx && f && stats, "null ctx/file/stats");
    FXG_LOCK(ctx);
    const int nranks = comm ? fxg_comm_nranks(comm) : 1, rank = comm ? fxg_comm_rank(comm) : 0;
    int rc = ctx->misc.reserve((size_t)nranks * sizeof(fxg_shard_info) + 256);
    if (rc) return rc;
    fxg_shard_info *d_all = (fxg_shard_info *)ctx->misc.ptr;
    if ((rc = fxg_scan_begin(ctx, f, mode, base_offset, flags, nullptr))) return rc;
    if ((rc = fxg_shard_exchange(ctx, comm, own_info(ctx), d_all, sizeof(fxg_shard_info)))) return rc;
    if ((rc = fxg_scan_finish(ctx, d_all, nranks, rank, d_rows_out, stats, all_host))) return rc;
    return comm ? fxg_comm_check(comm) : FXG_OK;
}

extern "C" int fxg_fasta_scan(fxg_ctx *ctx, const fxg_file *f, int64_t base_offset, int flags,
                              fxg_fasta_row **d_rows_out, fxg_scan_stats *stats) {
    FXG_CHECK_ARG(ctx && f && stats, "null ctx/file/stats");
    FXG_LOCK(ctx);
    int rc = fxg_scan_begin(ctx, f, 0, base_offset, flags, nullptr);
    if (rc) return rc;
    return fxg_scan_finish(ctx, nullptr, 1, 0, (void **)d_rows_out, stats, nullptr);
}

extern "C" int fxg_fastq_scan(fxg_ctx *ctx, const fxg_file *f, int64_t base_offset,
                              fxg_fastq_row **d_rows_out, fxg_scan_stats *stats) {
    FXG_CHECK_ARG(ctx && f && stats, "null ctx/file/stats");
    FXG_LOCK(ctx);
    int rc = fxg_scan_begin(ctx, f, 1, base_offset, 0, nullptr);
    if (rc) return rc;
    return fxg_scan_finish(ctx, nullptr, 1, 0, (void **)d_rows_out, stats, nullptr);
}

extern "C" int fxg_split_point_dev(fxg_ctx *ctx, const fxg_file *f, int64_t from, int want_header, int64_t *pos) {
    FXG_CHECK_ARG(ctx && f && pos && from >= 0, "bad arguments");
    FXG_LOCK(ctx);
    FXG_CUDA(cudaSetDevice(ctx->device));
    if (from >= f->size) { *pos = f->size; return FXG_OK; }
    int rc;
    if ((rc = ctx->counters.reserve(1024))) return rc;
    long long *d = (long long *)((uint8_t *)ctx->counters.ptr + 512);
    ctx->launches += 1;
    split_point_kernel<<<1, 256, 0, ctx->stream>>>(f->d, f->size, from, want_header, d);
    FXG_CUDA(cudaGetLastError());
    long long h = 0;
    FXG_CUDA(cudaMemcpyAsync(&h, d, 8, cudaMemcpyDeviceToHost, ctx->stream));
    FXG_CUDA(cudaStreamSynchronize(ctx->stream));
    *pos = (int64_t)h;
    return FXG_OK;
}
```

Baseline: 2373.

## Fuse FASTA prefix expansion into lines kernel and fold edge/shard-prefix kernels

For FASTA, the per-region prefix-expand pass and the ex array go away. fasta_lines_kernel now computes each region's exclusive prefix itself, with warp scans over 256-region groups seeded from a coarser block sum. The edge and shard-prefix kernels are merged into prefix_blocks_kernel and clear_kernel, which means fewer launches. prefix_blocks is rewritten to give each thread a contiguous chunk, mark_kernel's multi-region-per-warp loop is dropped, and a bandwidth-floor probe kernel is added. The change removes global traffic and launches, at the cost of more complex fused kernels and extra seg writes skipped for sparse regions.

```diff
diff --git a/include/fxg.h b/include/fxg.h
--- a/include/fxg.h
+++ b/include/fxg.h
@@ -115,6 +115,7 @@
 
 int fxg_scan_begin(fxg_ctx *ctx, const fxg_file *f, int mode, int64_t base_offset, int flags,
                    fxg_shard_info *d_info_out );
+int fxg_scan_floor(fxg_ctx *ctx, const fxg_file *f);
 int fxg_shard_exchange(fxg_ctx *ctx, fxg_comm *comm, const void *d_send, void *d_recv, int64_t bytes_per_rank);
 int fxg_scan_finish(fxg_ctx *ctx, const fxg_shard_info *d_all , int nranks, int rank,
                     void **d_rows_out, fxg_scan_stats *stats, fxg_shard_info *all_host);
diff --git a/pyfastx_b200/_cabi.py b/pyfastx_b200/_cabi.py
--- a/pyfastx_b200/_cabi.py
+++ b/pyfastx_b200/_cabi.py
@@ -90,6 +90,7 @@
     "fxg_fasta_scan": (i32, [vp, vp, i64, i32, P(vp), P(ScanStats)]),
     "fxg_fastq_scan": (i32, [vp, vp, i64, P(vp), P(ScanStats)]),
     "fxg_scan_begin": (i32, [vp, vp, i32, i64, i32, vp]),
+    "fxg_scan_floor": (i32, [vp, vp]),
     "fxg_shard_exchange": (i32, [vp, vp, vp, vp, i64]),
     "fxg_scan_finish": (i32, [vp, vp, i32, i32, P(vp), P(ScanStats), vp]),
     "fxg_scan_sharded": (i32, [vp, vp, vp, i32, i64, i32, P(vp), P(ScanStats), vp]),
@@ -156,6 +157,8 @@
                                        "__graft_entry__.build()); there is no CPU fallback")
         L = C.CDLL(LIB_PATH)
         for name, (res, args) in SIGNATURES.items():
+            if os.environ.get("FXG_LIB_PATH") and not hasattr(L, name):
+                continue
             fn = getattr(L, name)
             fn.restype = res
             fn.argtypes = args
diff --git a/pyfastx_b200/csrc/fxg_scan.cu b/pyfastx_b200/csrc/fxg_scan.cu
--- a/pyfastx_b200/csrc/fxg_scan.cu
+++ b/pyfastx_b200/csrc/fxg_scan.cu
@@ -105,14 +105,8 @@
     return 255u;
 }
 
-#ifndef FXG_MARK_V_FASTA
-#define FXG_MARK_V_FASTA 1
-#endif
 #ifndef FXG_MARK_V_FASTQ
 #define FXG_MARK_V_FASTQ 2
-#endif
-#ifndef FXG_MARK_RPW
-#define FXG_MARK_RPW 1
 #endif
 __device__ __forceinline__ uint32_t swz_unit(uint32_t u) { return u ^ ((u >> 3) & 7u); }
 template <int V>
@@ -125,24 +119,25 @@
     __shared__ uint4    s_data[MARK_WARPS * (REGION / 16) + (FXG_MARK_CUT ? 2 : 0)];
     __shared__ uint16_t s_ent[MARK_WARPS][SEGCAP];
     const int lane = threadIdx.x & 31, warp = threadIdx.x >> 5;
-    const int64_t r0 = ((int64_t)blockIdx.x * MARK_WARPS + warp) * FXG_MARK_RPW;
-    if (r0 >= P.nreg) return;
+    const int64_t r = (int64_t)blockIdx.x * MARK_WARPS + warp;
+    if (r >= P.nreg) return;
     const uint32_t lt_mask = (1u << lane) - 1u;
     const int64_t n = P.n;
     const uint8_t *file = P.file;
     const uint32_t k0a = reg_const(0x0a0a0a0au), k7f = reg_const(0x7f7f7f7fu), k80 = reg_const(0x80808080u);
 
-    auto load_region = [&](int64_t rr, uint4 (&vv)[4]) {
-        const int64_t base = rr * REGION;
+    const int64_t base = r * REGION;
+    uint4 v[4];
+    {
         if (base + REGION <= n) {
             const uint8_t *src = file + base + lane * 16;
 #pragma unroll
-            for (int j = 0; j < 4; ++j) vv[j] = ld_stream16(src + j * 512);
+            for (int j = 0; j < 4; ++j) v[j] = ld_stream16(src + j * 512);
         } else {
 #pragma unroll
             for (int j = 0; j < 4; ++j) {
                 const int64_t o = base + j * 512 + lane * 16;
-                if (o + 16 <= n) { vv[j] = ld_stream16(file + o); continue; }
+                if (o + 16 <= n) { v[j] = ld_stream16(file + o); continue; }
                 const bool virt = n > 0 && file[n - 1] != '\n';
                 uint32_t w[4] = {0, 0, 0, 0};
                 for (int i = 0; i < 16; ++i) {
@@ -150,19 +145,10 @@
                     const uint32_t b = x < n ? file[x] : ((virt && x == n) ? 0x0au : 0u);
                     w[i >> 2] |= b << ((i & 3) * 8);
                 }
-                vv[j] = make_uint4(w[0], w[1], w[2], w[3]);
-            }
-        }
-    };
-    uint4 vn[4];
-    load_region(r0, vn);
-#pragma unroll 1
-    for (int it = 0; it < FXG_MARK_RPW; ++it) {
-    const int64_t r = r0 + it;
-    if (r >= P.nreg) break;
-    const int64_t base = r * REGION;
-    uint4 v[4] = {vn[0], vn[1], vn[2], vn[3]};
-    if (it + 1 < FXG_MARK_RPW && r + 1 < P.nreg) load_region(r + 1, vn);
+                v[j] = make_uint4(w[0], w[1], w[2], w[3]);
+            }
+        }
+    }
     uint32_t nlc = 0;
     uint16_t *ent = s_ent[warp];
 
@@ -322,7 +308,8 @@
                     hmask = hb;
                 }
             }
-            if (k < nround) dst[k] = (uint16_t)e;
+            const bool keep = MODE == 1 || nlc > 32u || imask != 0u;
+            if (keep && k < nround) dst[k] = (uint16_t)e;
             if (FXG_MARK_CUT && MODE == 1) P.cut[r * SEGCAP + k] = (uint8_t)cutv;
             if (k < nlc) ent[k] = (uint16_t)e;
         }
@@ -331,8 +318,8 @@
             const uint32_t last = nlc >= 1 ? ent[nlc - 1] : 0u, prev = nlc >= 2 ? ent[nlc - 2] : 0u;
             P.rc[r] = make_uint2(nlc | (hc << 16), last | (prev << 16));
             if (MODE == 0) {
-                const uint32_t f0 = nlc >= 1 ? ent[0] : 0u, f1 = nlc >= 2 ? ent[1] : 0u;
-                P.rec2[r] = make_uint4(f0 | (f1 << 16), nlc > 32u ? 0xffffffffu : imask, hmask, 0u);
+                const uint32_t f0 = nlc >= 1 ? ent[0] : 0u, f1 = nlc >= 2 ? ent[1] : 0u, f2 = nlc >= 3 ? ent[2] : 0u;
+                P.rec2[r] = make_uint4(f0 | (f1 << 16), nlc > 32u ? 0xffffffffu : imask, hmask, f2);
             }
         }
     } else {
@@ -350,11 +337,26 @@
             if (MODE == 0) P.rec2[r] = make_uint4(0u, 0xffffffffu, 0u, 0u);
         }
     }
-    __syncwarp();
-    }
-}
-
+}
+
+__global__ void __launch_bounds__(MARK_WARPS * 32, FXG_MARK_MINB) mark_floor_kernel(const uint8_t *file, int64_t n,
+                                                                                    uint32_t *sink) {
+    const int lane = threadIdx.x & 31;
+    const int64_t base = ((int64_t)blockIdx.x * MARK_WARPS + (threadIdx.x >> 5)) * REGION;
+    if (base + REGION > n) return;
+    uint4 v[4];
+#pragma unroll
+    for (int j = 0; j < 4; ++j) v[j] = ld_stream16(file + base + j * 512 + lane * 16);
+    uint32_t x = 0;
+#pragma unroll
+    for (int j = 0; j < 4; ++j) x ^= v[j].x ^ v[j].y ^ v[j].z ^ v[j].w;
+    x = __reduce_xor_sync(0xffffffffu, x);
+    if (lane == 0 && x == 0x9e3779b9u) atomicAdd(sink, 1u);
+}
+
+template <int GROUP>
 __global__ void __launch_bounds__(PS_THREADS) prefix_reduce_kernel(const uint2 *rc, ulonglong2 *bs) {
+    static_assert(GROUP == 256 || GROUP == PS_BLOCK, "group size");
     __shared__ uint32_t sm[16];
     const uint4 *p = reinterpret_cast<const uint4 *>(rc + (size_t)blockIdx.x * PS_BLOCK + (size_t)threadIdx.x * PS_PER_THREAD);
     uint32_t a = 0, b = 0;
@@ -364,9 +366,15 @@
         a += (q.x & 0xffffu) + (q.z & 0xffffu);
         b += (q.x >> 16) + (q.z >> 16);
     }
+    const int lane = threadIdx.x & 31, warp = threadIdx.x >> 5;
+    if (GROUP == 256) {
+#pragma unroll
+        for (int d = 8; d > 0; d >>= 1) { a += __shfl_xor_sync(0xffffffffu, a, d); b += __shfl_xor_sync(0xffffffffu, b, d); }
+        if ((lane & 15) == 0) bs[((size_t)blockIdx.x * PS_THREADS + threadIdx.x) / 16] = make_ulonglong2(a, b);
+        return;
+    }
     a = __reduce_add_sync(0xffffffffu, a);
     b = __reduce_add_sync(0xffffffffu, b);
-    const int lane = threadIdx.x & 31, warp = threadIdx.x >> 5;
     if (lane == 0) { sm[warp] = a; sm[8 + warp] = b; }
     __syncthreads();
     if (threadIdx.x == 0) {
@@ -376,36 +384,100 @@
     }
 }
 
-__global__ void __launch_bounds__(1024) prefix_blocks_kernel(ulonglong2 *bs, int64_t nb, const uint8_t *file, int64_t n,
-                                                             int mode, ScanTotals *tot) {
+__device__ __forceinline__ bool nl_at(const ScanParams &P, int64_t x);
+__device__ void shard_edge(const ScanParams &P, int mode, const ScanTotals &t, fxg_shard_info *info) {
+    const int lane = threadIdx.x & 31;
+    int found = 0;
+    int64_t pos[3] = {0, 0, 0};
+    for (int64_t r0 = 0; r0 < P.nreg && found < 3; r0 += 32) {
+        const int64_t r = r0 + lane;
+        const uint32_t c = r < P.nreg ? (P.rc[r].x & 0xffffu) : 0u;
+        uint32_t nz = __ballot_sync(0xffffffffu, c != 0);
+        while (nz && found < 3) {
+            const int fl = __ffs(nz) - 1;
+            nz &= nz - 1;
+            const int64_t q = r0 + fl;
+            const int cq = (int)__shfl_sync(0xffffffffu, c, fl);
+            if (cq <= SEGCAP) {
+                const uint4 f = mode == 0 ? P.rec2[q] : make_uint4(0u, 0u, 0u, 0u);
+                for (int i = 0; i < cq && found < 3; ++i) {
+                    const uint32_t e = mode != 0 ? (uint32_t)P.seg[q * SEGCAP + i] : (i == 0 ? f.x : i == 1 ? f.x >> 16 : f.w);
+                    pos[found++] = q * REGION + (int64_t)(e & E_POS);
+                }
+            } else {
+                for (int64_t x = q * REGION; x < q * REGION + REGION && found < 3; ++x)
+                    if (nl_at(P, x)) pos[found++] = x;
+            }
+        }
+    }
+    if (lane == 0) {
+        fxg_shard_info o;
+        o.n_rows = mode == 0 ? (int64_t)t.hdr : 0;
+        o.n_lines = (int64_t)t.nl;
+        o.bytes = P.n;
+        o.base_offset = P.base_offset;
+        o.end_position = t.n_eff;
+        o.edge_n = found;
+        int64_t start = 0;
+        for (int j = 0; j < 3; ++j) {
+            o.edge_off[j] = 0; o.edge_len[j] = 0;
+            if (j < found) {
+                const int64_t p = pos[j];
+                const bool cr = p > start && p - 1 < P.n && P.file[p - 1] == '\r';
+                o.edge_off[j] = P.base_offset + start;
+                o.edge_len[j] = p - start - (cr ? 1 : 0);
+                start = p + 1;
+            }
+        }
+        for (int j = 0; j < 4; ++j) o.reserved[j] = 0;
+        *info = o;
+    }
+}
+
+__global__ void __launch_bounds__(1024) prefix_blocks_kernel(const ScanParams P, int64_t nb, int mode, fxg_shard_info *info) {
     __shared__ uint64_t s_a[32], s_b[32];
-    __shared__ uint64_t s_ca, s_cb;
+    __shared__ ScanTotals s_t;
+    ulonglong2 *bs = P.bs;
+    const int64_t n = P.n;
     const int lane = threadIdx.x & 31, warp = threadIdx.x >> 5;
-    if (threadIdx.x == 0) { s_ca = 0; s_cb = (mode == 0 && n > 0 && file[0] == '>') ? 1u : 0u; }
+    const int64_t per = (nb + 1023) / 1024, i0 = min(nb, (int64_t)threadIdx.x * per), i1 = min(nb, i0 + per);
+    uint64_t ta = 0, tb = 0;
+    for (int64_t i = i0; i < i1; i += 8) {
+        ulonglong2 v[8];
+#pragma unroll
+        for (int j = 0; j < 8; ++j) v[j] = i + j < i1 ? bs[i + j] : make_ulonglong2(0, 0);
+#pragma unroll
+        for (int j = 0; j < 8; ++j) { ta += v[j].x; tb += v[j].y; }
+    }
+    uint64_t a = ta, b = tb;
+#pragma unroll
+    for (int d = 1; d < 32; d <<= 1) {
+        const uint64_t oa = (uint64_t)shfl_up_i64((int64_t)a, d), ob = (uint64_t)shfl_up_i64((int64_t)b, d);
+        if (lane >= d) { a += oa; b += ob; }
+    }
+    if (lane == 31) { s_a[warp] = a; s_b[warp] = b; }
     __syncthreads();
-    for (int64_t b0 = 0; b0 < nb; b0 += 1024) {
-        const int64_t i = b0 + threadIdx.x;
-        const ulonglong2 v = i < nb ? bs[i] : make_ulonglong2(0, 0);
-        uint64_t a = v.x, b = v.y;
-#pragma unroll
-        for (int d = 1; d < 32; d <<= 1) {
-            const uint64_t oa = (uint64_t)shfl_up_i64((int64_t)a, d), ob = (uint64_t)shfl_up_i64((int64_t)b, d);
-            if (lane >= d) { a += oa; b += ob; }
-        }
-        if (lane == 31) { s_a[warp] = a; s_b[warp] = b; }
-        __syncthreads();
-        uint64_t wa = 0, wb = 0;
-        for (int w = 0; w < warp; ++w) { wa += s_a[w]; wb += s_b[w]; }
-        const uint64_t ca = s_ca, cb = s_cb;
-        if (i < nb) bs[i] = make_ulonglong2(ca + wa + a - v.x, cb + wb + b - v.y);
-        __syncthreads();
-        if (threadIdx.x == 1023) { s_ca = ca + wa + a; s_cb = cb + wb + b; }
-        __syncthreads();
-    }
-    if (threadIdx.x == 0) {
-        const bool virt = n > 0 && file[n - 1] != '\n';
-        tot->nl = s_ca; tot->hdr = s_cb; tot->n_eff = n + (virt ? 1 : 0);
-    }
+    uint64_t ea = a - ta, eb = (mode == 0 && n > 0 && P.file[0] == '>') ? 1u : 0u;
+    eb += b - tb;
+    for (int w = 0; w < warp; ++w) { ea += s_a[w]; eb += s_b[w]; }
+    for (int64_t i = i0; i < i1; i += 8) {
+        ulonglong2 v[8];
+#pragma unroll
+        for (int j = 0; j < 8; ++j) v[j] = i + j < i1 ? bs[i + j] : make_ulonglong2(0, 0);
+#pragma unroll
+        for (int j = 0; j < 8; ++j) {
+            if (i + j < i1) bs[i + j] = make_ulonglong2(ea, eb);
+            ea += v[j].x; eb += v[j].y;
+        }
+    }
+    if (threadIdx.x == 1023) {
+        const bool virt = n > 0 && P.file[n - 1] != '\n';
+        memset(&s_t, 0, sizeof(s_t));
+        s_t.nl = ea; s_t.hdr = eb; s_t.n_eff = n + (virt ? 1 : 0);
+        P.totals->nl = s_t.nl; P.totals->hdr = s_t.hdr; P.totals->n_eff = s_t.n_eff;
+    }
+    __syncthreads();
+    if (warp == 0) shard_edge(P, mode, s_t, info);
 }
 
 __global__ void __launch_bounds__(PS_THREADS) prefix_expand_kernel(const uint2 *rc, const ulonglong2 *bs, ulonglong2 *ex,
@@ -576,16 +648,17 @@
     int64_t q = r - 1;
     while (need > 0 && q >= 0) {
         const int64_t qq = q - lane;
-        const uint32_t c = qq >= 0 ? (P.rc[qq].x & 0xffffu) : 0u;
+        const uint2 rec = qq >= 0 ? P.rc[qq] : make_uint2(0u, 0u);
+        const uint32_t c = rec.x & 0xffffu;
         const uint32_t nz = __ballot_sync(0xffffffffu, c != 0);
         if (!nz) { q -= 32; continue; }
         const int f = __ffs(nz) - 1;
         q -= f;
         const int cq = (int)__shfl_sync(0xffffffffu, c, f);
         if (cq <= SEGCAP) {
-            const uint16_t *sg = P.seg + q * SEGCAP;
-            for (int i = cq - 1; i >= 0 && need > 0; --i) {
-                const uint32_t e = sg[i];
+            const uint32_t y = __shfl_sync(0xffffffffu, rec.y, f);
+            for (int i = 0; i < 2 && i < cq && need > 0; ++i) {
+                const uint32_t e = (y >> (16 * i)) & 0xffffu;
                 push(q * REGION + (int64_t)(e & E_POS), MODE == 0 ? (e >> 15) : 0u);
             }
         } else {
@@ -684,13 +757,12 @@
 }
 
 template <int MODE>
-__device__ __noinline__ unsigned long long full_region(const ScanParams *Pg, int64_t first_line, int64_t r) {
+__device__ __noinline__ unsigned long long full_region(const ScanParams *Pg, int64_t first_line, int64_t r, ulonglong2 X) {
     const ScanParams &P = *Pg;
     unsigned long long my_size = 0;
     const int lane = threadIdx.x & 31;
     const int nl = (int)(P.rc[r].x & 0xffffu);
     if (nl == 0) return 0;
-    const ulonglong2 X = P.ex[r];
     Prev2 cy = carry_walk<MODE>(Pg, r);
     if (MODE != 0) cy.h1 = cy.h0 = 0;
     if (nl <= SEGCAP) region_batches<MODE>(P, first_line, r, nl, cy, X, P.seg[r * SEGCAP + lane], P.seg[r * SEGCAP + 32 + lane], my_size);
@@ -802,7 +874,7 @@
     const uint32_t densem = __ballot_sync(0xffffffffu, nll > (uint32_t)SEGCAP);
     if (densem & (((1u << RG) - 1u) << 1)) {
         for (int i = 0; i < RG; ++i)
-            if (r0 + i < P.nreg) my_size += full_region<1>(P.self, first_line, r0 + i);
+            if (r0 + i < P.nreg) my_size += full_region<1>(P.self, first_line, r0 + i, P.ex[r0 + i]);
     } else {
         const uint64_t ex0 = (uint64_t)shfl_i64((int64_t)exl, 1);
         uint16_t *flat = s_flat[warp];
@@ -942,53 +1014,92 @@
     if (lane == 0 && my_size) atomicAdd((unsigned long long *)&P.totals->sum_len, my_size);
 }
 
-__global__ void __launch_bounds__(MARK_WARPS * 32) fasta_lines_kernel(const ScanParams P) {
-    const int lane = threadIdx.x & 31;
-    const int64_t R0 = ((int64_t)blockIdx.x * MARK_WARPS + (threadIdx.x >> 5)) * 32;
-    if (R0 >= P.nreg) return;
+constexpr int FL_REGIONS = MARK_WARPS * 32;
+static_assert(FL_REGIONS == 256 && PS_BLOCK % FL_REGIONS == 0, "rows CTA = one prefix group");
+__global__ void __launch_bounds__(FL_REGIONS) fasta_lines_kernel(const ScanParams P) {
+    __shared__ uint32_t s_a[MARK_WARPS], s_b[MARK_WARPS];
+    const int lane = threadIdx.x & 31, warp = threadIdx.x >> 5;
+    const int64_t R0 = (int64_t)blockIdx.x * FL_REGIONS + warp * 32;
     const int64_t r = R0 + lane;
     const bool inb = r < P.nreg;
     unsigned long long dummy = 0;
-    uint2 me = make_uint2(0u, 0u), pv = make_uint2(0u, 0u);
+    uint2 me = make_uint2(0u, 0u);
     uint4 q = make_uint4(0u, 0u, 0u, 0u);
-    ulonglong2 X = make_ulonglong2(0, 0);
     if (inb) {
         me = P.rc[r];
-        if (r >= 1) pv = P.rc[r - 1];
         q = P.rec2[r];
-        X = P.ex[r];
-    }
-    const uint32_t nl = me.x & 0xffffu, pnl = pv.x & 0xffffu;
-    const bool full = nl != 0 && (nl > 32u || r == 0 || pnl < 2u || pnl > (uint32_t)SEGCAP || q.y == 0xffffffffu);
+    }
+    uint2 pv = make_uint2(__shfl_up_sync(0xffffffffu, me.x, 1), __shfl_up_sync(0xffffffffu, me.y, 1));
+    if (lane == 0 && inb && r >= 1) pv = P.rc[r - 1];
+    const uint32_t nl = me.x & 0xffffu, pnl = pv.x & 0xffffu, hc = me.x >> 16;
+    uint32_t ia = nl, ib = hc;
+#pragma unroll
+    for (int d = 1; d < 32; d <<= 1) {
+        const uint32_t oa = __shfl_up_sync(0xffffffffu, ia, d), ob = __shfl_up_sync(0xffffffffu, ib, d);
+        if (lane >= d) { ia += oa; ib += ob; }
+    }
+    if (lane == 31) { s_a[warp] = ia; s_b[warp] = ib; }
+    __syncthreads();
+    const ulonglong2 g = P.bs[blockIdx.x];
+    ulonglong2 X = make_ulonglong2(g.x + ia - nl, g.y + ib - hc);
+    for (int w = 0; w < warp; ++w) { X.x += s_a[w]; X.y += s_b[w]; }
+    if (R0 >= P.nreg) return;
+
+    const bool full = nl > 32u;
+    const uint32_t f0 = q.x & 0xffffu, f1 = q.x >> 16;
+    const int64_t base = r * REGION;
+    Prev2 cy;
+    cy.pos1 = cy.pos0 = NOPOS; cy.h1 = cy.h0 = 0;
+    bool walk = false;
+    if (nl != 0 && !full) {
+        if (r == 0) { cy.pos1 = -1; cy.h1 = is_hdr_at<0>(P, 0); }
+        else if (pnl >= 2u && pnl <= (uint32_t)SEGCAP) {
+            const uint32_t c1 = pv.y & 0xffffu, c0 = pv.y >> 16;
+            cy.pos1 = base - REGION + (c1 & E_POS); cy.h1 = c1 >> 15;
+            cy.pos0 = base - REGION + (c0 & E_POS); cy.h0 = c0 >> 15;
+        } else walk = true;
+    }
+    uint32_t wm = __ballot_sync(0xffffffffu, walk);
+    while (wm) {
+        const int f = __ffs(wm) - 1;
+        wm &= wm - 1;
+        const Prev2 c = carry_walk<0>(P.self, R0 + f);
+        if (lane == f) cy = c;
+    }
     uint32_t mask = 0;
-    const uint32_t c1 = pv.y & 0xffffu, c0 = pv.y >> 16, f0 = q.x & 0xffffu, f1 = q.x >> 16;
     if (nl != 0 && !full) {
-        const int p_c1 = (int)(c1 & E_POS) - REGION, p_c0 = (int)(c0 & E_POS) - REGION;
-        const int p_f0 = (int)(f0 & E_POS), p_f1 = (int)(f1 & E_POS);
-        const int L0 = p_f0 - p_c1;
-        const bool i0 = ((c1 | c0) & E_HDR) != 0 || L0 != p_c1 - p_c0;
-        const bool i1 = nl >= 2u && (((f0 | c1) & E_HDR) != 0 || p_f1 - p_f0 != L0);
+        const int64_t p_f0 = base + (f0 & E_POS), p_f1 = base + (f1 & E_POS);
+        const int64_t L0 = p_f0 - cy.pos1;
+        const bool i0 = cy.h1 != 0 || cy.h0 != 0 || cy.pos1 < 0 || L0 != cy.pos1 - cy.pos0;
+        const bool i1 = nl >= 2u && ((f0 & E_HDR) != 0 || cy.h1 != 0 || p_f1 - p_f0 != L0);
         mask = (q.y & ~3u) | (i0 ? 1u : 0u) | (i1 ? 2u : 0u);
         if (nl < 32u) mask &= (1u << nl) - 1u;
     }
-    const int64_t base = r * REGION;
     const uint16_t *sg = P.seg + r * SEGCAP;
     while (mask) {
         const int k = __ffs(mask) - 1;
         mask &= mask - 1;
-        uint32_t e, m1, m2;
-        int64_t b1 = base, b2 = base;
-        if (k >= 2) { e = sg[k]; m1 = sg[k - 1]; m2 = sg[k - 2]; }
-        else if (k == 1) { e = f1; m1 = f0; m2 = c1; b2 = base - REGION; }
-        else { e = f0; m1 = c1; m2 = c0; b1 = b2 = base - REGION; }
-        do_line<0>(P, 0, base + (e & E_POS), b1 + (m1 & E_POS), b2 + (m2 & E_POS), (m1 & E_HDR) != 0, (m2 & E_HDR) != 0,
-                   (int64_t)X.y + __popc(q.z & ((1u << k) - 1u)), (int64_t)X.x + k, false, dummy);
+        int64_t p, pm1, pm2;
+        bool h1, h2;
+        if (k >= 2) {
+            const uint32_t e = sg[k], m1 = sg[k - 1], m2 = sg[k - 2];
+            p = base + (e & E_POS); pm1 = base + (m1 & E_POS); pm2 = base + (m2 & E_POS);
+            h1 = (m1 & E_HDR) != 0; h2 = (m2 & E_HDR) != 0;
+        } else if (k == 1) {
+            p = base + (f1 & E_POS); pm1 = base + (f0 & E_POS); pm2 = cy.pos1;
+            h1 = (f0 & E_HDR) != 0; h2 = cy.h1 != 0;
+        } else {
+            p = base + (f0 & E_POS); pm1 = cy.pos1; pm2 = cy.pos0;
+            h1 = cy.h1 != 0; h2 = cy.h0 != 0;
+        }
+        do_line<0>(P, 0, p, pm1, pm2, h1, h2, (int64_t)X.y + __popc(q.z & ((1u << k) - 1u)), (int64_t)X.x + k, false, dummy);
     }
     uint32_t fm = __ballot_sync(0xffffffffu, full);
     while (fm) {
         const int f = __ffs(fm) - 1;
         fm &= fm - 1;
-        full_region<0>(P.self, 0, R0 + f);
+        const ulonglong2 Xf = make_ulonglong2((uint64_t)shfl_i64((int64_t)X.x, f), (uint64_t)shfl_i64((int64_t)X.y, f));
+        full_region<0>(P.self, 0, R0 + f, Xf);
     }
 }
 
@@ -1040,54 +1151,7 @@
     }
 }
 
-__global__ void __launch_bounds__(32) edge_kernel(const ScanParams P, int mode, fxg_shard_info *info) {
-    const int lane = threadIdx.x;
-    int found = 0;
-    int64_t pos[3] = {0, 0, 0};
-    for (int64_t r0 = 0; r0 < P.nreg && found < 3; r0 += 32) {
-        const int64_t r = r0 + lane;
-        const uint32_t c = r < P.nreg ? (P.rc[r].x & 0xffffu) : 0u;
-        uint32_t nz = __ballot_sync(0xffffffffu, c != 0);
-        while (nz && found < 3) {
-            const int fl = __ffs(nz) - 1;
-            nz &= nz - 1;
-            const int64_t q = r0 + fl;
-            const int cq = (int)__shfl_sync(0xffffffffu, c, fl);
-            if (cq <= SEGCAP) {
-                for (int i = 0; i < cq && found < 3; ++i) pos[found++] = q * REGION + (int64_t)(P.seg[q * SEGCAP + i] & E_POS);
-            } else {
-                for (int64_t x = q * REGION; x < q * REGION + REGION && found < 3; ++x)
-                    if (nl_at(P, x)) pos[found++] = x;
-            }
-        }
-    }
-    if (lane == 0) {
-        const ScanTotals t = *P.totals;
-        fxg_shard_info o;
-        o.n_rows = mode == 0 ? (int64_t)t.hdr : 0;
-        o.n_lines = (int64_t)t.nl;
-        o.bytes = P.n;
-        o.base_offset = P.base_offset;
-        o.end_position = t.n_eff;
-        o.edge_n = found;
-        int64_t start = 0;
-        for (int j = 0; j < 3; ++j) {
-            o.edge_off[j] = 0; o.edge_len[j] = 0;
-            if (j < found) {
-                const int64_t p = pos[j];
-                const bool cr = p > start && p - 1 < P.n && P.file[p - 1] == '\r';
-                o.edge_off[j] = P.base_offset + start;
-                o.edge_len[j] = p - start - (cr ? 1 : 0);
-                start = p + 1;
-            }
-        }
-        for (int j = 0; j < 4; ++j) o.reserved[j] = 0;
-        *info = o;
-    }
-}
-
-__global__ void shard_prefix_kernel(const fxg_shard_info *all, int nranks, int rank, int mode, ScanTotals *tot) {
-    if (threadIdx.x != 0 || blockIdx.x != 0) return;
+__device__ void shard_prefix(const fxg_shard_info *all, int nranks, int rank, int mode, ScanTotals *tot) {
     int64_t F = 0, T = 0;
     for (int p = 0; p < nranks; ++p) {
         const int64_t nlp = all[p].n_lines;
@@ -1101,12 +1165,17 @@
     tot->nrows = mode == 0 ? (int64_t)tot->hdr : (F + nl + 3) / 4 - F / 4;
     tot->sum_len = 0;
 }
-
-__global__ void __launch_bounds__(256) clear_kernel(const ScanParams P, int mode, int64_t tmp_slots) {
-    const int64_t nrows = P.totals->nrows;
+__global__ void shard_prefix_kernel(const fxg_shard_info *all, int nranks, int rank, int mode, ScanTotals *tot) {
+    if (threadIdx.x == 0 && blockIdx.x == 0) shard_prefix(all, nranks, rank, mode, tot);
+}
+
+__global__ void __launch_bounds__(256) clear_kernel(const ScanParams P, int mode, int64_t tmp_slots, const fxg_shard_info *all,
+                                                    int nranks, int rank) {
+    const int64_t nrows = mode == 0 ? (int64_t)P.totals->hdr : P.totals->nrows;
     const int64_t stride = (int64_t)gridDim.x * blockDim.x;
     const int64_t t0 = (int64_t)blockIdx.x * blockDim.x + threadIdx.x;
     if (mode == 0) {
+        if (t0 == 0) shard_prefix(all, nranks, rank, mode, P.totals);
         int64_t slots = nrows + 2;
         if (slots > tmp_slots) slots = tmp_slots;
         uint4 *p = reinterpret_cast<uint4 *>(P.tmp);
@@ -1179,15 +1248,19 @@
 
 static int64_t guess_rows(int mode, int64_t n) { return (mode == 0 ? n / 1024 : n / 200) + 4096; }
 
+static int64_t prefix_groups(int mode, int64_t nreg) {
+    const int64_t nreg_pad = (nreg + PS_BLOCK - 1) / PS_BLOCK * PS_BLOCK;
+    return nreg_pad / (mode == 0 ? FL_REGIONS : PS_BLOCK);
+}
+
 static int scan_params(fxg_ctx *ctx, const fxg_file *f, int mode, int64_t base_offset, int flags, bool reserve,
                        ScanParams *out, int64_t *tmp_slots) {
     const int64_t n = f->size;
     const int64_t nreg = (n + 1 + REGION - 1) / REGION;
-    const int64_t nb = (nreg + PS_BLOCK - 1) / PS_BLOCK;
-    const int64_t nreg_pad = nb * PS_BLOCK;
+    const int64_t nreg_pad = (nreg + PS_BLOCK - 1) / PS_BLOCK * PS_BLOCK;
     const size_t off_bs = fxg_round_up((int64_t)nreg_pad * 8, 256);
-    const size_t off_ex = off_bs + fxg_round_up(nb * (int64_t)sizeof(ulonglong2), 256);
-    const size_t off_r2 = off_ex + fxg_round_up(nreg * (int64_t)sizeof(ulonglong2), 256);
+    const size_t off_ex = off_bs + fxg_round_up(prefix_groups(mode, nreg) * (int64_t)sizeof(ulonglong2), 256);
+    const size_t off_r2 = off_ex + (mode == 1 ? fxg_round_up(nreg * (int64_t)sizeof(ulonglong2), 256) : 0);
     int rc;
     if (reserve) {
         if ((rc = ctx->counters.reserve(1024))) return rc;
@@ -1208,8 +1281,8 @@
     P.base_offset = base_offset; P.first_line = 0; P.flags = flags;
     P.rc = (uint2 *)ctx->tile_desc.ptr;
     P.bs = (ulonglong2 *)((uint8_t *)ctx->tile_desc.ptr + off_bs);
-    P.ex = (ulonglong2 *)((uint8_t *)ctx->tile_desc.ptr + off_ex);
-    P.rec2 = (uint4 *)((uint8_t *)ctx->tile_desc.ptr + off_r2);
+    P.ex = mode == 1 ? (ulonglong2 *)((uint8_t *)ctx->tile_desc.ptr + off_ex) : nullptr;
+    P.rec2 = mode == 0 ? (uint4 *)((uint8_t *)ctx->tile_desc.ptr + off_r2) : nullptr;
     P.seg = (uint16_t *)ctx->seg.ptr;
     P.cut = (uint8_t *)ctx->cut.ptr;
     P.totals = (ScanTotals *)((uint8_t *)ctx->counters.ptr + 64);
@@ -1242,19 +1315,19 @@
     const int64_t nb = (nreg + PS_BLOCK - 1) / PS_BLOCK, nreg_pad = nb * PS_BLOCK;
     FXG_CUDA(cudaMemsetAsync(ctx->counters.ptr, 0, 1024, ctx->stream));
     if (nreg_pad > nreg) FXG_CUDA(cudaMemsetAsync(P.rc + nreg, 0, (size_t)(nreg_pad - nreg) * 8, ctx->stream));
-    const unsigned grid = (unsigned)((nreg + (int64_t)MARK_WARPS * FXG_MARK_RPW - 1) / ((int64_t)MARK_WARPS * FXG_MARK_RPW));
+    const unsigned grid = (unsigned)((nreg + MARK_WARPS - 1) / MARK_WARPS);
     {
         FxgProfScope prof(ctx, FXG_PROF_SCAN);
-        if (mode == 0) mark_kernel<0, FXG_MARK_V_FASTA><<<grid, MARK_WARPS * 32, 0, ctx->stream>>>(P);
+        if (mode == 0) mark_kernel<0, 1><<<grid, MARK_WARPS * 32, 0, ctx->stream>>>(P);
         else mark_kernel<1, FXG_MARK_V_FASTQ><<<grid, MARK_WARPS * 32, 0, ctx->stream>>>(P);
     }
     FXG_CUDA(cudaGetLastError());
     {
-        FxgProfScope prof(ctx, FXG_PROF_PREFIX, 4);
-        prefix_reduce_kernel<<<(unsigned)nb, PS_THREADS, 0, ctx->stream>>>(P.rc, P.bs);
-        prefix_blocks_kernel<<<1, 1024, 0, ctx->stream>>>(P.bs, nb, P.file, n, mode, P.totals);
-        prefix_expand_kernel<<<(unsigned)nb, PS_THREADS, 0, ctx->stream>>>(P.rc, P.bs, P.ex, nreg);
-        edge_kernel<<<1, 32, 0, ctx->stream>>>(P, mode, own_info(ctx));
+        FxgProfScope prof(ctx, FXG_PROF_PREFIX, mode == 0 ? 2 : 3);
+        if (mode == 0) prefix_reduce_kernel<FL_REGIONS><<<(unsigned)nb, PS_THREADS, 0, ctx->stream>>>(P.rc, P.bs);
+        else prefix_reduce_kernel<PS_BLOCK><<<(unsigned)nb, PS_THREADS, 0, ctx->stream>>>(P.rc, P.bs);
+        prefix_blocks_kernel<<<1, 1024, 0, ctx->stream>>>(P, prefix_groups(mode, nreg), mode, own_info(ctx));
+        if (mode == 1) prefix_expand_kernel<<<(unsigned)nb, PS_THREADS, 0, ctx->stream>>>(P.rc, P.bs, P.ex, nreg);
     }
     FXG_CUDA(cudaGetLastError());
     if (d_info_out)
@@ -1275,11 +1348,11 @@
     FXG_CUDA(cudaMemcpyAsync(ctx->params.ptr, (uint8_t *)ctx->h_counters + 4096, sizeof(P), cudaMemcpyHostToDevice, ctx->stream));
     const int64_t nreg = P.nreg;
     {
-        FxgProfScope prof(ctx, FXG_PROF_LINES, 3);
-        shard_prefix_kernel<<<1, 32, 0, ctx->stream>>>(d_all, nranks, rank, mode, P.totals);
-        clear_kernel<<<ctx->sm_count * 4, 256, 0, ctx->stream>>>(P, mode, tmp_slots);
+        FxgProfScope prof(ctx, FXG_PROF_LINES, mode == 0 ? 2 : 3);
+        if (mode == 1) shard_prefix_kernel<<<1, 32, 0, ctx->stream>>>(d_all, nranks, rank, mode, P.totals);
+        clear_kernel<<<ctx->sm_count * 4, 256, 0, ctx->stream>>>(P, mode, tmp_slots, d_all, nranks, rank);
         if (mode == 0) {
-            const unsigned lgrid = (unsigned)((nreg + MARK_WARPS * 32 - 1) / (MARK_WARPS * 32));
+            const unsigned lgrid = (unsigned)((nreg + FL_REGIONS - 1) / FL_REGIONS);
             fasta_lines_kernel<<<lgrid, MARK_WARPS * 32, 0, ctx->stream>>>(P);
         } else if (getenv("FXG_FASTQ_LINES_GENERIC")) {
             const unsigned lgrid = (unsigned)((nreg + MARK_WARPS * LG - 1) / (MARK_WARPS * LG));
@@ -1390,6 +1463,24 @@
     return fxg_scan_finish(ctx, nullptr, 1, 0, (void **)d_rows_out, stats, nullptr);
 }
 
+extern "C" int fxg_scan_floor(fxg_ctx *ctx, const fxg_file *f) {
+    FXG_CHECK_ARG(ctx && f, "null ctx/file");
+    FXG_LOCK(ctx);
+    FXG_CUDA(cudaSetDevice(ctx->device));
+    int rc;
+    if ((rc = ctx->counters.reserve(1024))) return rc;
+    const int64_t nreg = f->size / REGION;
+    if (nreg == 0) return FXG_OK;
+    {
+        FxgProfScope prof(ctx, FXG_PROF_SCAN);
+        const size_t smem = MARK_WARPS * (REGION + SEGCAP * sizeof(uint16_t));
+        mark_floor_kernel<<<(unsigned)((nreg + MARK_WARPS - 1) / MARK_WARPS), MARK_WARPS * 32, smem, ctx->stream>>>(
+            f->d, f->size, (uint32_t *)((uint8_t *)ctx->counters.ptr + 768));
+    }
+    FXG_CUDA(cudaGetLastError());
+    return FXG_OK;
+}
+
 extern "C" int fxg_split_point_dev(fxg_ctx *ctx, const fxg_file *f, int64_t from, int want_header, int64_t *pos) {
     FXG_CHECK_ARG(ctx && f && pos && from >= 0, "bad arguments");
     FXG_LOCK(ctx);
```

Measured after the change: 2553 (median of 6 runs). +7.6%, better.
